# uber/aresdb

Hardware: AMD Instinct MI355X
Metric: rows/sec, 1B-row filter -> group-by-agg (whole job) (higher is better)
Workload: dtype u32 keys / f64 sums; 1 GPU; C3: filter d1<90 -> dims [floor(ts,3600), d1, d2, d3] (4 x uint32) -> SUM(m float32 -> float64) via HashReduce, validity bitmaps with 1% nulls, shard resident in HBM; rows_per_gpu=1000000000, batch_rows=67108864, batches=15, streams_per_query=2, parallelism=1 shard(s), one per GPU

## Files before the change

aresdb_amd/abi.py:

```python
import ctypes as C
import os

_HERE = os.path.dirname(os.path.abspath(__file__))
REPO_ROOT = os.path.dirname(_HERE)
LIB_DIR = os.environ.get("ARES_LIB_DIR") or os.path.join(_HERE, "lib")

AGGR_SUM_UNSIGNED, AGGR_SUM_SIGNED, AGGR_SUM_FLOAT = 1, 2, 3
AGGR_MIN_UNSIGNED, AGGR_MIN_SIGNED, AGGR_MIN_FLOAT = 4, 5, 6
AGGR_MAX_UNSIGNED, AGGR_MAX_SIGNED, AGGR_MAX_FLOAT = 7, 8, 9
AGGR_HLL, AGGR_AVG_FLOAT = 10, 11

(Bool, Int8, Uint8, Int16, Uint16, Int32, Uint32, Float32, Int64, Uint64, Float64, GeoPoint,
 UUID) = range(13)
ConstInt, ConstFloat, ConstGeoPoint, ConstUUID = range(4)
(Negate, Not, BitwiseNot, IsNull, IsNotNull, Noop, GetWeekStart, GetMonthStart, GetQuarterStart,
 GetYearStart, GetDayOfMonth, GetDayOfYear, GetMonthOfYear, GetQuarterOfYear, GetHLLValue,
 ArrayLength) = range(16)
(And, Or, Equal, NotEqual, LessThan, LessThanOrEqual, GreaterThan, GreaterThanOrEqual, Plus, Minus,
 Multiply, Divide, Mod, BitwiseAnd, BitwiseOr, BitwiseXor, Floor, ArrayContains,
 ArrayElementAt) = range(19)
(VectorPartyInput, ScratchSpaceInput, ConstantInput, ForeignColumnInput,
 ArrayVectorPartyInput) = range(5)
ScratchSpaceOutput, MeasureOutput, DimensionOutput = range(3)
NUM_DIM_WIDTH = 5
# ... 231 lines not shown
        return _check(getattr(self, "_" + sym)(*args))

    def mem_driver_calls(self, device=0):
        if not hasattr(self._mem, "AresMemDriverCalls"):
            return None
        m, f, t = C.c_size_t(0), C.c_size_t(0), C.c_size_t(0)
        self._mem.AresMemDriverCalls.argtypes = [C.c_int, C.POINTER(C.c_size_t), C.POINTER(C.c_size_t), C.POINTER(C.c_size_t)]
        self._mem.AresMemDriverCalls.restype = None
        self._mem.AresMemDriverCalls(device, C.byref(m), C.byref(f), C.byref(t))
        return {"mallocs": m.value, "frees": f.value, "trims": t.value}

    def rtc_wait(self):
        if not hasattr(self._algo, "AresRtcWait"):
            return None
        c = (C.c_long * 3)()
        self._algo.AresRtcWait.argtypes, self._algo.AresRtcWait.restype = [C.POINTER(C.c_long)], C.c_size_t
        n = self._algo.AresRtcWait(c)
        return {"kernels": int(n), "compiles": int(c[0]), "disk_hits": int(c[1]), "evictions": int(c[2])}

    def reload_env(self):
        if hasattr(self._algo, "AresReloadEnv"):
            self._algo.AresReloadEnv.argtypes, self._algo.AresReloadEnv.restype = [], None
            self._algo.AresReloadEnv()

    def flags(self):
        return self._mem.GetFlags()

    @property
    def has_fused_select(self):
        return hasattr(self._algo, "AresFusedFilterSelect")

    def fused_filter_select(self, query, batch_rows, limit, out_keys, stream=None, device=0):
        fn = self._algo.AresFusedFilterSelect
        fn.argtypes = [C.POINTER(FusedSelect), C.c_int, C.c_int, DimensionVector, _S, _I]
        fn.restype = CGoCallResHandle
        return _check(fn(C.byref(query), int(batch_rows), int(limit), out_keys, stream, device))

    def select_stats(self):
        c = (C.c_ulonglong * 4)()
        self._algo.AresSelectStats.argtypes, self._algo.AresSelectStats.restype = [C.POINTER(C.c_ulonglong)], None
        self._algo.AresSelectStats(c)
        return {"batches": int(c[0]), "declined": int(c[1]), "tiles": int(c[2]), "rows": int(c[3])}

    @property
    def has_fused_join_select(self):
        return hasattr(self._algo, "AresFusedFilterJoinSelect")

    def fused_filter_join_select(self, query, batch_rows, limit, out_keys, stream=None, device=0):
        fn = self._algo.AresFusedFilterJoinSelect
        fn.argtypes = [C.POINTER(FusedJoinSelect), C.c_int, C.c_int, DimensionVector, _S, _I]
        fn.restype = CGoCallResHandle
        return _check(fn(C.byref(query), int(batch_rows), int(limit), out_keys, stream, device))

    def select_join_stats(self):
        c = (C.c_ulonglong * 5)()
        self._algo.AresSelectJoinStats.argtypes, self._algo.AresSelectJoinStats.restype = [C.POINTER(C.c_ulonglong)], None
        self._algo.AresSelectJoinStats(c)
        return {"batches": int(c[0]), "declined": int(c[1]), "tiles": int(c[2]), "rows": int(c[3]), "probed": int(c[4])}

    @property
    def has_join_columns(self):
        return hasattr(self._algo, "AresJoinColumnsRun")

    def join_column_bytes(self, rows, dtype):
        fn = self._algo.AresJoinColumnBytes
        fn.argtypes, fn.restype = [C.c_int, C.c_int], C.c_size_t
        return int(fn(int(rows), int(dtype)))

    def join_columns_run(self, query, batch_rows, stream=None, device=0):
        fn = self._algo.AresJoinColumnsRun
        fn.argtypes = [C.POINTER(JoinColumns), C.c_int, C.POINTER(VectorPartySlice), _S, _I]
        fn.restype = CGoCallResHandle
        slices = (VectorPartySlice * 4)()
        res = _check(fn(C.byref(query), int(batch_rows), slices, stream, device))
        assert res == batch_rows
        return slices

    def join_column_stats(self):
        c = (C.c_ulonglong * 4)()
        self._algo.AresJoinColumnStats.argtypes, self._algo.AresJoinColumnStats.restype = [C.POINTER(C.c_ulonglong)], None
        self._algo.AresJoinColumnStats(c)
        return {"batches": int(c[0]), "declined": int(c[1]), "rows": int(c[2]), "probed": int(c[3])}

    def select_run_stats(self):
        c = (C.c_ulonglong * 2)()
        self._algo.AresSelectRunStats.argtypes, self._algo.AresSelectRunStats.restype = [C.POINTER(C.c_ulonglong)], None
        self._algo.AresSelectRunStats(c)
        return {"rejected": int(c[0]), "staged": int(c[1])}

    def profiler_enable(self, on=True):
        self._algo.AresProfilerEnable(1 if on else 0)

    def profiler_report(self):
        need = self._algo.AresProfilerReport(None, 0)
        buf = C.create_string_buffer(need + 16)
        self._algo.AresProfilerReport(buf, need + 16)
        out = {}
        for line in buf.value.decode().splitlines():
            name, launches, ms = line.rsplit(" ", 2)
            out[name] = (int(launches), float(ms))
        return out

    def device_alloc(self, nbytes, device=0):
        return self.call("DeviceAllocate", max(int(nbytes), 1), device)

    def device_free(self, ptr, device=0):
        self.call("DeviceFree", ptr, device)

    def h2d(self, dst, src_buf, nbytes, stream=None, device=0):
        self.call("AsyncCopyHostToDevice", dst, src_buf, nbytes, stream, device)

    def d2h(self, dst_buf, src, nbytes, stream=None, device=0):
        self.call("AsyncCopyDeviceToHost", dst_buf, src, nbytes, stream, device)

    def wait(self, stream=None, device=0):
        self.call("WaitForCudaStream", stream, device)


def hip_library_paths():
    return os.path.join(LIB_DIR, "libalgorithm.so"), os.path.join(LIB_DIR, "libmem.so")


def load_hip_backend():
    if not os.environ.get("ARES_NO_TORCH"):
        import torch
    algo, mem = hip_library_paths()
    return Backend("hip", algo, mem, device_memory=True)
```

aresdb_amd/csrc/algo/common.hpp:

```cpp
#pragma once

#include <hip/hip_runtime.h>

#include <atomic>
#include <chrono>
#include <cstdint>
#include <cstdio>
#include <cstdlib>
#include <cstring>
#include <stdexcept>
#include <string>

#include "ares_algorithm.h"

namespace ares {

class AlgorithmError : public std::runtime_error {
 public:
  explicit AlgorithmError(const std::string &m) : std::runtime_error(m) {}
};

void slow_trace(const char *what, double ms);
bool hr_trace_enabled();
class SlowScope {
 public:
  explicit SlowScope(const char *what) : what_(what), t0_(std::chrono::steady_clock::now()) {}
  ~SlowScope() {
    const double ms = std::chrono::duration<double, std::milli>(std::chrono::steady_clock::now() - t0_).count();
    if (ms > 5.0) slow_trace(what_, ms);
  }
  SlowScope(const SlowScope &) = delete;
  SlowScope &operator=(const SlowScope &) = delete;

 private:
  const char *what_;
  std::chrono::steady_clock::time_point t0_;
};
inline void hip_check(hipError_t e, const char *what) {
  if (e != hipSuccess) {
    (void)hipGetLastError();
    throw AlgorithmError(std::string("ERROR: ") + what + ": " + hipGetErrorString(e));
  }
}

template <class F>
inline void hip_check_timed(F &&call, const char *what) {
  SlowScope slow(what);
  hip_check(call(), what);
}
#define hip_check(expr, what) hip_check_timed([&]() -> hipError_t { return (expr); }, what)

extern void (*g_memNoteActivity)();
inline void mem_note_activity() {
  if (g_memNoteActivity) g_memNoteActivity();
}
inline void check_launch(const char *what) {
  mem_note_activity();
  hip_check(hipGetLastError(), what);
}

void flush_deferred(int device);
bool fuse_pending_into_hash_reduce(int device, hipStream_t stream, const DimensionVector &in, const uint8_t *inValues,
                                   const DimensionVector &out, uint8_t *outValues, int valueBytes, int length, int aggFunc,
                                   int *groups);
void invalidate_filter_journal(int device, const uint32_t *indexVector);
bool global_table_forced();
bool deferral_hooks_active();
void grouped_note_write(int device, const void *ptr, size_t bytes);
void grouped_note_write(int device, const DimensionVector &v);
void grouped_materialize_for_read(int device, const void *ptr, size_t bytes);
void grouped_trim(int device);
void flush_deferred_for_inputs(int device, const void *a, size_t aBytes, const void *b, size_t bBytes);
void flush_deferred_for_vector(int device, const DimensionVector &v, const void *values, size_t valueBytes);
void drop_skipped_outputs(int device, const void *a, size_t aBytes, const void *b, size_t bBytes);

bool defer_fill(int device, hipStream_t stream, void *dst, size_t bytes, uint64_t pattern, int unit);
bool pending_fill_exact(int device, const void *dst, size_t bytes, uint64_t *pattern, int *unit);
bool pending_fill_tail(int device, const void *base, int width, int length, int *prev, uint64_t *pattern);
void retire_fills_for_write(int device, const void *ptr, size_t bytes);
void materialize_fills_for_read(int device, const void *ptr, size_t bytes);
void launch_pending_writers(int device, const void *ptr, size_t bytes);
bool virtual_iota_peek(int device, const uint32_t *indexVector, int n, bool consume = false);
void materialize_index_vector(int device, const uint32_t *indexVector);
void settle_dimension_vector(int device, const DimensionVector &v, bool rowsOnly = false);
void temp_stats(size_t *handedOut, size_t *cached);

struct CallStream {
  hipStream_t stream;
  bool known;
};
extern thread_local CallStream t_callStream;
class CallStreamScope {
 public:
  CallStreamScope(void *stream, const char *entry) : saved_(t_callStream), slow_(entry) {
    t_callStream = CallStream{reinterpret_cast<hipStream_t>(stream), true};
  }
  ~CallStreamScope() { t_callStream = saved_; }
  CallStreamScope(const CallStreamScope &) = delete;
  CallStreamScope &operator=(const CallStreamScope &) = delete;

 private:
  CallStream saved_;
  SlowScope slow_;
};

#define ARES_ABI_BEGIN_NOFLUSH(device)                 \
  CGoCallResHandle resHandle = {nullptr, nullptr};     \
  try {                                                \
    ares::hip_check(hipSetDevice(device), "hipSetDevice");  \
    ares::CallStreamScope callStreamScope_(cudaStream, __func__);  \
    ares::mem_note_activity();                                      \
    (void)ares::deferral_hooks_active();

#define ARES_ABI_BEGIN(device)     \
  ARES_ABI_BEGIN_NOFLUSH(device)   \
  ares::flush_deferred(device);

#define ARES_ABI_END(name)                                            \
  }                                                                   \
  catch (std::exception & e) {                                        \
    fprintf(stderr, "Exception happened when doing %s: %s\n", name, e.what()); \
    resHandle.pStrErr = strdup(e.what());                             \
  }                                                                   \
  return resHandle;

extern std::atomic<uint32_t> g_envGeneration;
template <typename T>
class EnvSwitch {
 public:
  EnvSwitch(const char *name, T (*parse)(const char *)) : name_(name), parse_(parse) {}
  T get() {
    const uint32_t g = g_envGeneration.load(std::memory_order_acquire);
    if (gen_.load(std::memory_order_acquire) != g) {
      value_.store(parse_(getenv(name_)), std::memory_order_relaxed);
      gen_.store(g, std::memory_order_release);
    }
    return value_.load(std::memory_order_relaxed);
  }

 private:
  const char *name_;
  T (*parse_)(const char *);
  std::atomic<uint32_t> gen_{0};
  std::atomic<T> value_{};
};

inline void *int_result(int64_t v) { return reinterpret_cast<void *>(static_cast<intptr_t>(v)); }

// ... 66 lines not shown
```

aresdb_amd/csrc/algo/hash_reduce.hip:

```cpp
#include <hip/hip_runtime.h>

#include "aggregate.hpp"
#include "common.hpp"
#include "device_model.hpp"
#include "dim_layout.hpp"
#include "hash_reduce_lds.hpp"

namespace ares {

constexpr int kBlock = 256;
constexpr uint64_t kEmptyKey = ~0ull;

__global__ __launch_bounds__(kBlock) void hash_table_init_kernel(uint64_t *keys, uint8_t *values, uint64_t capacity,
                                                                 AggSpec a) {
  for (uint64_t s = static_cast<uint64_t>(blockIdx.x) * kBlock + threadIdx.x; s < capacity;
       s += static_cast<uint64_t>(gridDim.x) * kBlock) {
    keys[s] = kEmptyKey;
    if (a.width == 8) reinterpret_cast<uint64_t *>(values)[s] = a.identity;
    else reinterpret_cast<uint32_t *>(values)[s] = static_cast<uint32_t>(a.identity);
  }
}

__device__ __forceinline__ uint64_t find_or_claim(uint64_t *keys, uint64_t mask, uint32_t h, uint32_t row) {
  const uint64_t mine = (static_cast<uint64_t>(h) << 32) | row;
// ... 13 lines not shown
  }
}

__global__ __launch_bounds__(kBlock) void hash_insert_kernel(const uint8_t *dimValues, DimLayoutD L, size_t capacity,
                                                             const uint8_t *inputValues, AggSpec a, uint64_t *keys,
                                                             uint8_t *values, uint64_t mask, int length) {
  for (int64_t i64 = static_cast<int64_t>(blockIdx.x) * kBlock + threadIdx.x; i64 < length;
       i64 += static_cast<int64_t>(gridDim.x) * kBlock) {
    const uint32_t row = static_cast<uint32_t>(i64);
    Murmur32Stream ms(0);
    hash_dim_row(ms, dimValues, L, capacity, row);
    const uint32_t h = ms.finish();
    const uint64_t slot = find_or_claim(keys, mask, h, row);
    aggregate_slot(values + slot * a.width, inputValues + static_cast<size_t>(a.width) * row, a);
  }
}

constexpr int kExItems = 16;
__global__ __launch_bounds__(kBlock) void hash_extract_kernel(const uint64_t *keys, const uint8_t *values,
                                                              uint64_t tableSize, const uint8_t *dimIn, uint8_t *dimOut,
                                                              DimLayoutD L, size_t capacity, uint8_t *outputValues,
                                                              AggSpec a, uint32_t *counter) {
  __shared__ uint32_t sWave[kBlock / 64];
  __shared__ uint32_t sBase;
  const int lane = threadIdx.x & 63, wave = threadIdx.x >> 6;
  const uint64_t tileSlots = static_cast<uint64_t>(kBlock) * kExItems;
  for (uint64_t base = blockIdx.x * tileSlots; base < tableSize; base += gridDim.x * tileSlots) {
    uint64_t k[kExItems];
    uint32_t cnt = 0;
#pragma unroll
    for (int it = 0; it < kExItems; it++) {
      const uint64_t s = base + static_cast<uint64_t>(it) * kBlock + threadIdx.x;
      k[it] = s < tableSize ? keys[s] : kEmptyKey;
      cnt += k[it] != kEmptyKey;
    }
    uint32_t incl = cnt;
#pragma unroll
    for (int off = 1; off < 64; off <<= 1) {
      const uint32_t t = __shfl_up(incl, off);
      if (lane >= off) incl += t;
    }
    if (lane == 63) sWave[wave] = incl;
    __syncthreads();
    if (threadIdx.x == 0) {
      uint32_t total = 0;
      for (int w = 0; w < kBlock / 64; w++) {
        const uint32_t c = sWave[w];
        sWave[w] = total;
        total += c;
      }
      sBase = total ? atomicAdd(counter, total) : 0u;
    }
    __syncthreads();
    uint32_t dst = sBase + sWave[wave] + incl - cnt;
#pragma unroll
    for (int it = 0; it < kExItems; it++) {
      if (k[it] == kEmptyKey) continue;
      const uint64_t s = base + static_cast<uint64_t>(it) * kBlock + threadIdx.x;
      copy_dim_row(dimIn, capacity, dimOut, capacity, L, static_cast<uint32_t>(k[it]), dst);
      if (a.width == 8) reinterpret_cast<uint64_t *>(outputValues)[dst] = reinterpret_cast<const uint64_t *>(values)[s];
      else reinterpret_cast<uint32_t *>(outputValues)[dst] = reinterpret_cast<const uint32_t *>(values)[s];
      dst++;
    }
    __syncthreads();
  }
}

}

using namespace ares;

namespace ares {
bool global_table_forced() {
  static EnvSwitch<bool> forced("ARES_HASH_REDUCE", [](const char *e) { return e && strcmp(e, "global") == 0; });
  return forced.get();
}
}

extern "C" CGoCallResHandle HashReduce(DimensionVector inputKeys, uint8_t *inputValues, DimensionVector outputKeys,
                                       uint8_t *outputValues, int valueBytes, int length,
                                       enum AggregateFunction aggFunc, void *cudaStream, int device) {
  ARES_ABI_BEGIN_NOFLUSH(device)
  hipStream_t stream = reinterpret_cast<hipStream_t>(cudaStream);
  if (length > 0) {
    settle_dimension_vector(device, inputKeys);
    const DimLayoutD inLayout = make_dim_layout(inputKeys.NumDimsPerDimWidth);
    const size_t cap = inputKeys.VectorCapacity > 0 ? static_cast<size_t>(inputKeys.VectorCapacity) : 0;
    materialize_fills_for_read(device, inputKeys.DimValues, static_cast<size_t>(inLayout.rowBytes) * cap);
    materialize_fills_for_read(device, inputValues, static_cast<size_t>(valueBytes) * length);
    retire_fills_for_write(device, outputKeys.DimValues, static_cast<size_t>(inLayout.rowBytes) * cap);
    retire_fills_for_write(device, outputValues, static_cast<size_t>(valueBytes) * length);
  }
  {
    const DimLayoutD outLayout = make_dim_layout(outputKeys.NumDimsPerDimWidth);
    drop_skipped_outputs(device, outputKeys.DimValues,
                         static_cast<size_t>(outLayout.rowBytes) * (inputKeys.VectorCapacity > 0 ? inputKeys.VectorCapacity : 0),
                         outputValues, static_cast<size_t>(valueBytes) * (length > 0 ? length : 0));
  }
  int fusedGroups = 0;
  if (length > 0 && fuse_pending_into_hash_reduce(device, stream, inputKeys, inputValues, outputKeys, outputValues,
                                                  valueBytes, length, aggFunc, &fusedGroups)) {
    resHandle.res = int_result(fusedGroups);
    return resHandle;
  }
  {
    const DimLayoutD layout = make_dim_layout(inputKeys.NumDimsPerDimWidth);
    flush_deferred_for_inputs(device, inputKeys.DimValues, static_cast<size_t>(layout.rowBytes) * inputKeys.VectorCapacity,
                              inputValues, static_cast<size_t>(valueBytes) * (length > 0 ? length : 0));
  }
  const AggSpec a = make_agg_spec(aggFunc, valueBytes);
  int groups = -1;
  if (length > 0 && hash_reduce_lds_supported(a) && !global_table_forced())
    groups = hash_reduce_lds(device, inputKeys, inputValues, outputKeys, outputValues, a, length, stream);
  if (groups >= 0) {
    resHandle.res = int_result(groups);
  } else if (length > 0) {
    const DimLayoutD L = make_dim_layout(inputKeys.NumDimsPerDimWidth);
    grouped_note_write(device, outputValues, static_cast<size_t>(a.width) * length);
    grouped_note_write(device, outputKeys.DimValues, static_cast<size_t>(L.rowBytes) * inputKeys.VectorCapacity);
    uint64_t tableSize = 1024;
    while (tableSize < 2ull * static_cast<uint64_t>(length)) tableSize <<= 1;
    StreamBuffer keyBuf(tableSize * 8, stream), valBuf(tableSize * a.width, stream), counter(16, stream);
    hip_check(hipMemsetAsync(counter.get(), 0, 16, stream), "hipMemsetAsync");
    const int initGrid = capped_grid(static_cast<int64_t>((tableSize + kBlock - 1) / kBlock), 256 * 16);
    ARES_LAUNCH("hash_table_init_kernel", hash_table_init_kernel, initGrid, kBlock, stream, keyBuf.as<uint64_t>(),
                       valBuf.as<uint8_t>(), tableSize, a);
    const int grid = capped_grid((static_cast<int64_t>(length) + kBlock - 1) / kBlock, 256 * 16);
    ARES_LAUNCH("hash_insert_kernel", hash_insert_kernel, grid, kBlock, stream, inputKeys.DimValues, L,
                       static_cast<size_t>(inputKeys.VectorCapacity), inputValues, a, keyBuf.as<uint64_t>(),
                       valBuf.as<uint8_t>(), tableSize - 1, length);
    const int exGrid = capped_grid(static_cast<int64_t>((tableSize + kBlock * kExItems - 1) / (kBlock * kExItems)), 256 * 8);
    ARES_LAUNCH("hash_extract_kernel", hash_extract_kernel, exGrid, kBlock, stream, keyBuf.as<uint64_t>(),
                       valBuf.as<uint8_t>(), tableSize, inputKeys.DimValues, outputKeys.DimValues, L,
                       static_cast<size_t>(inputKeys.VectorCapacity), outputValues, a, counter.as<uint32_t>());
    uint32_t groups = 0;
    read_back_u32(counter.as<uint32_t>(), &groups, 1, stream);
    mem_note_dim_rows(device, outputKeys, 0, groups);
    mem_note_write(device, outputValues, static_cast<size_t>(a.width) * groups);
    resHandle.res = int_result(groups);
  }
  ARES_ABI_END("HashReduce")
}
```

aresdb_amd/csrc/algo/hash_reduce_lds.hip:

```cpp
#include <hip/hip_runtime.h>

#include <atomic>
#include <functional>
#include <map>
#include <mutex>
#include <string>
#include <unordered_map>

#include <memory>
#include <mutex>
#include <vector>

#include "aggregate.hpp"
#include "common.hpp"
#include "device_model.hpp"
#include "ares_extensions.h"
#include "dim_layout.hpp"
#include "fast_eval.hpp"
#include "hash_reduce_lds.hpp"
#include "hr_kernels.hpp"
#include "hr_rtc.hpp"
#include "sort_reduce_fused.hpp"

namespace ares {
// ... 599 lines not shown
    if (imageMode == 1) imageOut = take_image(device);
    if (prevSize > 0) grouped_materialize_for_read(device, prevValues, static_cast<size_t>(mw) * prevSize);
  }
  if (imageMode && !imageOut) {
    imageMode = 0;
    knownOut = 0;
    if (prevSize > 0) grouped_materialize_for_read(device, prevValues, static_cast<size_t>(mw) * prevSize);
  }
  {
    if (hr_trace_enabled())
      fprintf(stderr, "fused_hash_reduce_run: batch %d prev %d partBits %d | found %d (state: size %d partBits %d ranges %d image %d lazy %d) grouped %d "
                      "| lean %d table %d compact %d narrow %d -> image mode %d knownOut %u\n",
              batchRows, prevSize, partBits, found ? 1 : 0, found ? prev.size : -1, found ? prev.partBits : -1, found && prev.ranges ? 1 : 0,
              found && prev.image ? 1 : 0, found && prev.lazyValues ? 1 : 0, grouped ? 1 : 0, lean ? 1 : 0, table ? 1 : 0, compact ? 1 : 0,
              narrow ? 1 : 0, imageMode, knownOut);
  }
  if (narrow && !imageMode) {
    narrowMerge = rtc_lookup(device, rtc_spec_merge(plan, nd, partBits, a, widen, wantLean && compact,
                                                    wantTable || (prevSize > 0 && !grouped)));
    if (!narrowMerge) return kFusedUnavailable;
  }
  if (narrow && !(wantLean ? lean : table)) return kFusedUnavailable;
  bool launched = false;
  for (;;) {
    const bool prevToA = narrow && prevSize > 0 && !grouped && imageMode != 2;
    if (narrow && !imageMode) {
      narrowMerge = rtc_lookup(device, rtc_spec_merge(plan, nd, partBits, a, widen, lean && compact, table || prevToA));
      if (!narrowMerge) return launched ? -1 : kFusedUnavailable;
      if (table) tableMerge = narrowMerge;
    }
    launched = true;
    const int streams = batchRows > 0 ? (lean ? rtc_scan_grid(batchRows) : table ? 0 : grid_for(batchRows)) : 0;
    Regions r;
    {
      SlowScope slow("make_regions");
      const int64_t rowsA = !lean ? length : (prevSize > 0 && !grouped && imageMode != 2) ? prevSize : 0;
      make_regions(r, partBits, rowsA, batchRows, streams, lean ? 4 : 3, stream,
                   !lean ? 0 : compact ? static_cast<int>(kCompactLineRecords) : 8);
    }
    Workspace &ws = r.ws;
    ws.widen = widen;
    ws.chunkRows = static_cast<uint32_t>(chunkTiles) * 4096u;
    ws.rowBase = static_cast<uint32_t>(prevSize);
    ws.prevRanges = (grouped && imageMode != 2) ? prev.ranges.get() : nullptr;
    ws.outRanges = outRanges;
    Workspace wsPrev = ws;
    wsPrev.streams = 0;
    RtcKernel leanMerge = imageMode ? imageMerge
                          : narrow  ? (lean ? narrowMerge : nullptr)
                          : (lean && (prevSize == 0 || grouped)) ? rtc_lookup(device, rtc_spec_merge(plan, nd, partBits, a, widen, compact)) : nullptr;
    RtcImageArgs imageArgs{nullptr, nullptr, nullptr, nullptr, 0u};
    if (imageMode) {
      imageArgs.in = imageMode == 2 ? prev.image.get() : nullptr;
      imageArgs.inCount = imageMode == 2 ? image_counts(prev.image.get()) : nullptr;
      imageArgs.out = imageOut.get();
      imageArgs.outCount = image_counts(imageOut.get());
      imageArgs.knownOut = knownOut;
    }
    const RtcImageArgs *imagePtr = imageMode ? &imageArgs : nullptr;
    if (prevToA) {
      const DimLayoutD prevLayout = make_dim_layout(prevKeys.NumDimsPerDimWidth);
      const int64_t tiles = (static_cast<int64_t>(prevSize) + kTileRows - 1) / kTileRows;
      ARES_LAUNCH("hr_partition_kernel", hr_partition_kernel, static_cast<int>(tiles < 256 ? tiles : 256), kThreads, stream,
                  prevKeys.DimValues, prevLayout, prevCapacity, prevValues, a, prevSize, wsPrev);
    }
    if (outRanges && !leanMerge && !tableMerge) hip_check(hipMemsetAsync(outRanges, 0, kRangesBytes, stream), "hipMemsetAsync");
#define ARES_FUSED_CASE(ND)                                                                                            \
  case ND:                                                                                                             \
    if (prevSize > 0 && !grouped && !narrow && imageMode != 2) {                                                       \
      if (mw == 8)                                                                                                     \
        ARES_LAUNCH("hr_partition4_kernel", (hr_partition4_kernel<ND, 8>), grid_for(prevSize), kThreads, stream,        \
                    prevKeys.DimValues, prevCapacity, prevValues, 0u, a, prevSize, wsPrev, 0);                         \
      else                                                                                                             \
        ARES_LAUNCH("hr_partition4_kernel", (hr_partition4_kernel<ND, 4>), grid_for(prevSize), kThreads, stream,        \
                    prevKeys.DimValues, prevCapacity, prevValues, 0u, a, prevSize, wsPrev, 0);                         \
    }                                                                                                                  \
    if (batchRows > 0 && lean)                                                                                         \
      rtc_scan_launch(lean, leanKind, plan, static_cast<uint32_t>(prevSize), batchRows, ws, stream);                   \
    else if (batchRows > 0 && table)                                                                                   \
      rtc_scan_launch(table, RTC_SCAN_TABLE, plan, static_cast<uint32_t>(prevSize), batchRows, ws, stream);            \
    else if (batchRows > 0)                                                                                            \
      ARES_LAUNCH("hr_fused_scan_kernel", hr_fused_scan_kernel<ND>, streams, kThreads, stream, plan,                   \
                  static_cast<uint32_t>(prevSize), a, batchRows, ws);                                                  \
    if (leanMerge || tableMerge)                                                                                       \
      rtc_merge_launch(leanMerge ? leanMerge : tableMerge, plan, prevKeys.DimValues, prevCapacity, prevValues,         \
                       static_cast<uint32_t>(prevSize), outKeys.DimValues, outCapacity, outValues, ws, stream, imagePtr, \
                       result_slot());                                                                                 \
    else if (lean)                                                                                                     \
      ARES_LAUNCH("hr_fused_merge_kernel", (hr_fused_merge_kernel<ND, 4>), numParts, kThreads, stream, plan,            \
                  prevKeys.DimValues, prevCapacity, prevValues, static_cast<uint32_t>(prevSize), outKeys.DimValues,    \
                  outCapacity, outValues, a, ws);                                                                      \
    else                                                                                                               \
      ARES_LAUNCH("hr_fused_merge_kernel", (hr_fused_merge_kernel<ND, 3>), numParts, kThreads, stream, plan,            \
                  prevKeys.DimValues, prevCapacity, prevValues, static_cast<uint32_t>(prevSize), outKeys.DimValues,    \
                  outCapacity, outValues, a, ws);                                                                      \
    break;
    switch (nd) {
      ARES_FUSED_CASE(1) ARES_FUSED_CASE(2) ARES_FUSED_CASE(3) ARES_FUSED_CASE(4)
      default:
        if (batchRows > 0 && lean) rtc_scan_launch(lean, leanKind, plan, static_cast<uint32_t>(prevSize), batchRows, ws, stream);
        else if (batchRows > 0 && table) rtc_scan_launch(table, RTC_SCAN_TABLE, plan, static_cast<uint32_t>(prevSize), batchRows, ws, stream);
        rtc_merge_launch(leanMerge ? leanMerge : tableMerge, plan, prevKeys.DimValues, prevCapacity, prevValues, static_cast<uint32_t>(prevSize),
                         outKeys.DimValues, outCapacity, outValues, ws, stream, imagePtr, result_slot());
        break;
    }
    {
      SlowScope slow("read_result");
      res = ((leanMerge || tableMerge) && result_slot()) ? read_result_pinned(stream) : read_result(ws, stream);
    }
    if (imageMode == 2) res.groups += static_cast<uint32_t>(prevSize);
    if (imageMode == 2) {
      if (res.groups > knownOut) mem_note_dim_rows(device, outKeys, knownOut, res.groups - knownOut);
    } else {
      mem_note_dim_rows(device, outKeys, 0, res.groups);
      mem_note_write(device, outValues, static_cast<size_t>(mw) * res.groups);
    }
    if ((narrow || imageMode == 2) && res.needGeneric) {
      r.buf->mark_idle();
      return -1;
    }
    if (imageMode == 1 && res.needGeneric) imageMode = 0;
    if (leanMerge && res.needGeneric && !res.overflow && !(grouped && res.stale)) {
      hip_check(hipMemsetAsync(ws.outCount, 0, 4 * sizeof(uint32_t), stream), "hipMemsetAsync");
      if (outRanges) hip_check(hipMemsetAsync(outRanges, 0, kRangesBytes, stream), "hipMemsetAsync");
      switch (nd) {
#define ARES_FUSED_REMERGE(ND)                                                                                         \
  case ND:                                                                                                             \
    ARES_LAUNCH("hr_fused_merge_kernel", (hr_fused_merge_kernel<ND, 4>), numParts, kThreads, stream, plan,              \
                prevKeys.DimValues, prevCapacity, prevValues, static_cast<uint32_t>(prevSize), outKeys.DimValues,      \
                outCapacity, outValues, a, ws);                                                                        \
    break;
        ARES_FUSED_REMERGE(1) ARES_FUSED_REMERGE(2) ARES_FUSED_REMERGE(3) ARES_FUSED_REMERGE(4)
#undef ARES_FUSED_REMERGE
      }
      res = read_result(ws, stream);
      mem_note_dim_rows(device, outKeys, 0, res.groups);
      mem_note_write(device, outValues, static_cast<size_t>(mw) * res.groups);
    }
#undef ARES_FUSED_CASE
    r.buf->mark_idle();
    if (grouped && res.stale) {
      grouped_note_write(device, prevKeys.DimValues, slots.row_bytes() * prevCapacity);
      grouped = false;
      imageMode = 0;
      continue;
    }
    if (res.overflow && lean && grow_record_stream_slack()) continue;
    break;
  }
  if (res.overflow) {
    return -1;
  }
  fused_note_first_batch(shape, static_cast<int>(res.groups));
  if (shape && !lean && !table) {
    if (static_cast<int>(res.groups) >= lean_min_groups()) {
      (void)rtc_lookup(device, rtc_spec_scan(plan, nd, partBits, compact));
      (void)rtc_lookup(device, rtc_spec_merge(plan, nd, partBits, a, widen, compact));
    } else {
      (void)rtc_lookup(device, rtc_spec_table_scan(plan, nd, partBits, a, widen));
    }
  }
  if (outRanges) {
    GroupedState s{device, outKeys.DimValues, outValues, outCapacity, slots, mw, static_cast<int>(res.groups), partBits, outRangesRef};
    if (imageMode == 2) {
      s.ranges = nullptr;
      s.image = imageOut;
      s.lineage = prev.lineage;
      s.gen = ++g_generation;
      s.parentGen = prev.gen;
      s.lazyValues = true;
    } else if (imageMode == 1) {
      s.image = imageOut;
      s.lineage = ++g_lineage;
      s.gen = ++g_generation;
    }
    if (res.groups > 0) grouped_register(s);
  }
  return static_cast<int>(res.groups);
}

namespace {

struct NotFusable : std::runtime_error {
  explicit NotFusable(const std::string &why) : std::runtime_error("not fusable: " + why) {}
// ... 78 lines not shown
```

aresdb_amd/csrc/algo/hll.hip:

```cpp
#include <dlfcn.h>
#include <hip/hip_runtime.h>

#include <atomic>
#include <cstring>
#include <string>

#include "ares_extensions.h"
#include "common.hpp"
#include "dim_layout.hpp"
#include "hash_reduce_lds.hpp"
#include "hr_kernels.hpp"
#include "hr_rtc.hpp"
#include "lookback.hpp"
#include "sort_reduce.hpp"

namespace ares {

namespace {

constexpr int kBlock = 256;

__device__ __forceinline__ bool hll_less(uint64_t h1, uint32_t v1, uint64_t h2, uint32_t v2) {
  return h1 == h2 ? v1 > v2 : h1 < h2;
}
// ... 541 lines not shown
  DimScanParams dp;
  dp.regStart = hp.regStart;
  dp.dims = dims;
  dp.registers = totals[1];
  dp.numTiles = dimTiles;
  dp.regCount = regCount;
  dp.ticket = reinterpret_cast<unsigned int *>(base2);
  dp.error = reinterpret_cast<uint32_t *>(base2) + 1;
  dp.status = reinterpret_cast<uint64_t *>(base2 + 64);
  dp.offsets = dp.status + dimTiles;
  ARES_LAUNCH("hll_dim_scan_kernel", hll_dim_scan_kernel, capped_grid(dimTiles), kBlock, stream, dp);
  uint32_t tail[2] = {0, 0};
  read_back_u32(reinterpret_cast<const uint32_t *>(dp.offsets + dims), tail, 2, stream);
  uint32_t err = 0;
  read_back_u32(dp.error, &err, 1, stream);
  if (err) throw AlgorithmError("ERROR: HyperLogLog: inter-tile scan timed out");
  const size_t total = static_cast<size_t>(tail[0]) | (static_cast<size_t>(tail[1]) << 32);

  uint8_t *hllVector = static_cast<uint8_t *>(result_alloc(total));
  *hllVectorPtr = hllVector;
  *hllVectorSizePtr = total;
  hip_check(hipMemsetAsync(hllVector, 0, total, stream), "hipMemsetAsync");
  ARES_LAUNCH("hll_write_kernel", hll_write_kernel, capped_grid((static_cast<int64_t>(n) + kBlock - 1) / kBlock, 256 * 8),
              kBlock, stream, cur.HashValues, curValues, n, hp.entryDim, hp.entryReg, hp.regStart, regCount, dp.offsets,
              hllVector);
  hip_check(hipMemcpyAsync(cur.IndexVector, hp.headIndex, sizeof(uint32_t) * static_cast<size_t>(dims),
                           hipMemcpyDeviceToDevice, stream), "hipMemcpyAsync");
  return dims;
}

int hyperloglog(const DimensionVector &prev, const DimensionVector &cur, uint32_t *prevValues, uint32_t *curValues,
                int prevResultSize, int curBatchSize, bool isLastBatch, uint8_t **hllVectorPtr,
                size_t *hllVectorSizePtr, uint16_t **regCountPtr, hipStream_t stream) {
  if (prevResultSize < 0 || curBatchSize < 0) throw std::invalid_argument("HyperLogLog: negative size");
  if (static_cast<int64_t>(prevResultSize) + curBatchSize >= (1ll << 30))
    throw std::invalid_argument("HyperLogLog supports up to 2^30 - 1 entries per call");
  const DimLayoutD L = make_dim_layout(cur.NumDimsPerDimWidth);
  const size_t capacity = static_cast<size_t>(cur.VectorCapacity);
  const int P = prevResultSize, n = curBatchSize;

  int runs = 0;
  if (n > 0) runs = hll_preagg_batch(prev, cur, prevValues, curValues, P, n, stream);
  if (n > 0 && runs < 0) {
    StreamBuffer positions(sizeof(uint32_t) * static_cast<size_t>(n), stream);
    sort_rows(prev.DimValues, L, capacity, cur.IndexVector, curValues, cur.HashValues, positions.as<uint32_t>(), true,
              n, stream);
    runs = hll_reduce_sorted(cur.HashValues, positions.as<uint32_t>(), cur.IndexVector, curValues, prev.HashValues + P,
                             prev.IndexVector + P, prevValues + P, n, stream);
  }
  int resSize = P + runs;
  if (resSize > 0) {
    const int tiles = (resSize + kMergeTile - 1) / kMergeTile;
    StreamBuffer split(sizeof(int) * (static_cast<size_t>(tiles) + 1), stream);
    ARES_LAUNCH("hll_merge_split_kernel", hll_merge_split_kernel, (tiles + 1 + kBlock - 1) / kBlock, kBlock, stream,
                prev.HashValues, prevValues, P, runs, tiles, split.as<int>());
    ARES_LAUNCH("hll_merge_kernel", hll_merge_kernel, tiles, kBlock, stream, prev.HashValues, prevValues,
                prev.IndexVector, P, runs, split.as<int>(), cur.HashValues, curValues, cur.IndexVector);
    if (isLastBatch)
      resSize = make_hll_vector(cur, curValues, resSize, hllVectorPtr, hllVectorSizePtr, regCountPtr, stream);
    ARES_LAUNCH("hll_gather_dims_kernel", hll_gather_dims_kernel,
                capped_grid((static_cast<int64_t>(resSize) + kBlock - 1) / kBlock, 256 * 8), kBlock, stream, prev.DimValues,
                cur.DimValues, make_dim_layout(prev.NumDimsPerDimWidth), static_cast<size_t>(prev.VectorCapacity),
                cur.IndexVector, resSize);
  }
  return resSize;
}

}

}

using namespace ares;

extern "C" void AresHllPreaggStats(unsigned long long *counters) {
  if (!counters) return;
  for (int i = 0; i < 4; i++) counters[i] = g_preaggStats[i].load(std::memory_order_relaxed);
}

extern "C" CGoCallResHandle HyperLogLog(DimensionVector prevDimOut, DimensionVector curDimOut, uint32_t *prevValuesOut,
                                        uint32_t *curValuesOut, int prevResultSize, int curBatchSize, bool isLastBatch,
                                        uint8_t **hllVectorPtr, size_t *hllVectorSizePtr,
                                        uint16_t **hllDimRegIDCountPtr, void *cudaStream, int device) {
  ARES_ABI_BEGIN(device)
  settle_dimension_vector(device, prevDimOut);
  settle_dimension_vector(device, curDimOut);
  {
    const size_t capV = static_cast<size_t>(prevDimOut.VectorCapacity > curDimOut.VectorCapacity ? prevDimOut.VectorCapacity : curDimOut.VectorCapacity);
    materialize_fills_for_read(device, prevValuesOut, 4 * capV);
    materialize_fills_for_read(device, curValuesOut, 4 * capV);
  }
  flush_deferred_for_vector(device, prevDimOut, nullptr, 0);
  flush_deferred_for_vector(device, curDimOut, nullptr, 0);
  grouped_note_write(device, prevDimOut);
  grouped_note_write(device, curDimOut);
  {
    mem_note_vector_all(device, prevDimOut);
    mem_note_vector_all(device, curDimOut);
    const size_t cap = static_cast<size_t>(prevDimOut.VectorCapacity > curDimOut.VectorCapacity ? prevDimOut.VectorCapacity
                                                                                                    : curDimOut.VectorCapacity);
    mem_note_write(device, prevValuesOut, 4 * cap);
    mem_note_write(device, curValuesOut, 4 * cap);
  }
  resHandle.res = reinterpret_cast<void *>(static_cast<intptr_t>(
      hyperloglog(prevDimOut, curDimOut, prevValuesOut, curValuesOut, prevResultSize, curBatchSize, isLastBatch,
                  hllVectorPtr, hllVectorSizePtr, hllDimRegIDCountPtr, reinterpret_cast<hipStream_t>(cudaStream))));
  ARES_ABI_END("HyperLogLog")
}
```

aresdb_amd/csrc/algo/sort_reduce.hip:

```cpp
#include <hip/hip_runtime.h>

#include "aggregate.hpp"
#include "common.hpp"
#include "device_model.hpp"
#include "dim_layout.hpp"
#include "lookback.hpp"
#include "sort_reduce_fused.hpp"

namespace ares {

constexpr int kBlock = 256;
constexpr int kWaves = kBlock / 64;

__global__ __launch_bounds__(kBlock) void sort_hash_hist_kernel(const uint8_t *dimValues, DimLayoutD L, size_t capacity,
                                                                const uint32_t *indexVector, uint64_t *hashes, int n,
                                                                uint32_t *globalHist ,
                                                                const uint32_t *hllValues, uint32_t *iotaOut) {
  __shared__ uint32_t sHist[8 * 256];
  for (int i = threadIdx.x; i < 8 * 256; i += kBlock) sHist[i] = 0;
  __syncthreads();
  for (int64_t i = static_cast<int64_t>(blockIdx.x) * kBlock + threadIdx.x; i < n;
       i += static_cast<int64_t>(gridDim.x) * kBlock) {
    Murmur128Stream ms(0);
    hash_dim_row(ms, dimValues, L, capacity, indexVector[i]);
// ... 826 lines not shown
    if (constRows) {
      uint64_t folded = constBits;
      if (a.op == OP_SUM) folded = (a.width == 8 ? constBits * static_cast<uint64_t>(constRows)
                                                 : static_cast<uint64_t>(static_cast<uint32_t>(constBits) * constRows));
      acc = combine_bits(a, acc, folded);
      any = true;
    }
  }
#pragma unroll
  for (int off = 32; off > 0; off >>= 1) {
    const uint64_t other = __shfl_xor(static_cast<unsigned long long>(acc), off);
    acc = combine_bits(a, acc, other);
  }
  if (__ballot(any) && (threadIdx.x & 63) == 0) aggregate_slot(out, reinterpret_cast<const uint8_t *>(&acc), a);
}

static bool reduce_without_dimensions(int device, const DimensionVector &in, const uint8_t *inputValues, const DimensionVector &out,
                                      uint8_t *outputValues, int valueBytes, int length, int aggFunc, hipStream_t stream, int *groups) {
  if (length <= 0) return false;
  const DimLayoutD L = make_dim_layout(in.NumDimsPerDimWidth), LO = make_dim_layout(out.NumDimsPerDimWidth);
  if (L.numDims != 0 || LO.numDims != 0 || aggFunc == AGGR_AVG_FLOAT) return false;
  AggSpec a;
  try {
    a = make_agg_spec(aggFunc, valueBytes);
  } catch (std::exception &) {
    return false;
  }
  if (!(a.vtype == V_U32 || a.vtype == V_I32 || a.vtype == V_U64 || a.vtype == V_I64)) return false;
  uint64_t hashPattern = 0;
  int hashUnit = 0;
  if (!in.HashValues || !in.IndexVector || !virtual_iota_peek(device, in.IndexVector, length) ||
      !pending_fill_exact(device, in.HashValues, 8ull * static_cast<size_t>(length), &hashPattern, &hashUnit) || hashUnit != 8)
    return false;
  int prev = length;
  uint64_t c = 0;
  if (!pending_fill_tail(device, inputValues, a.width, length, &prev, &c)) prev = length;
  if (prev > 0) {
    launch_pending_writers(device, inputValues, static_cast<size_t>(a.width) * prev);
    materialize_fills_for_read(device, inputValues, static_cast<size_t>(a.width) * prev);
  }
  retire_fills_for_write(device, outputValues, static_cast<size_t>(a.width));
  if (out.IndexVector) retire_fills_for_write(device, out.IndexVector, 4);
  mem_note_write(device, outputValues, static_cast<size_t>(a.width));
  if (out.IndexVector) mem_note_write(device, out.IndexVector, 4);
  (void)virtual_iota_peek(device, in.IndexVector, length, true);
  ARES_LAUNCH("fill_identity_kernel", fill_identity_kernel, 1, kBlock, stream, outputValues, a, 1);
  const int grid = capped_grid((static_cast<int64_t>(prev) + kBlock * 8 - 1) / (kBlock * 8), 256 * 4);
  ARES_LAUNCH("reduce_all_kernel", reduce_all_kernel, grid, kBlock, stream, inputValues, prev, a, c, static_cast<uint32_t>(length - prev),
              outputValues, out.IndexVector);
  *groups = 1;
  return true;
}

}

using namespace ares;

extern "C" {

CGoCallResHandle Sort(DimensionVector keys, int length, void *cudaStream, int device) {
  ARES_ABI_BEGIN_NOFLUSH(device)
  if (length > 0 && make_dim_layout(keys.NumDimsPerDimWidth).numDims == 0 && keys.HashValues && keys.IndexVector &&
      virtual_iota_peek(device, keys.IndexVector, length) &&
      defer_fill(device, reinterpret_cast<hipStream_t>(cudaStream), keys.HashValues, 8ull * static_cast<size_t>(length), empty_row_hash(), 8))
    return resHandle;
  if (define_lazy_sort(device, reinterpret_cast<hipStream_t>(cudaStream), keys, length)) return resHandle;
  const bool lazyVectors = lazy_vector_sort_candidate(device, keys, length);
  flush_deferred(device);
  settle_dimension_vector(device, keys, lazyVectors);
  flush_deferred_for_vector(device, keys, nullptr, 0);
  if (lazyVectors && define_lazy_sort_vectors(device, reinterpret_cast<hipStream_t>(cudaStream), keys, length)) return resHandle;
  if (length > 0) {
    mem_note_write(device, keys.HashValues, 8ull * static_cast<size_t>(length));
    mem_note_write(device, keys.IndexVector, 4ull * static_cast<size_t>(length));
  }
  sort_impl(keys, length, reinterpret_cast<hipStream_t>(cudaStream));
  ARES_ABI_END("Sort")
}

CGoCallResHandle Reduce(DimensionVector inputKeys, uint8_t *inputValues, DimensionVector outputKeys,
                        uint8_t *outputValues, int valueBytes, int length, enum AggregateFunction aggFunc,
                        void *cudaStream, int device) {
  ARES_ABI_BEGIN_NOFLUSH(device)
  {
    int groups = 0;
    if (reduce_without_dimensions(device, inputKeys, inputValues, outputKeys, outputValues, valueBytes, length, aggFunc,
                                  reinterpret_cast<hipStream_t>(cudaStream), &groups)) {
      resHandle.res = int_result(groups);
      return resHandle;
    }
  }
  {
    int groups = 0;
    if (length > 0 && fuse_pending_into_sort_reduce(device, reinterpret_cast<hipStream_t>(cudaStream), inputKeys, inputValues, outputKeys,
                                                    outputValues, valueBytes, length, aggFunc, &groups)) {
      resHandle.res = int_result(groups);
      return resHandle;
    }
  }
  flush_deferred(device);
  settle_dimension_vector(device, inputKeys);
  settle_dimension_vector(device, outputKeys);
  retire_fills_for_write(device, outputValues, static_cast<size_t>(valueBytes) * (length > 0 ? length : 0));
  flush_deferred_for_vector(device, inputKeys, inputValues, static_cast<size_t>(valueBytes) * (length > 0 ? length : 0));
  grouped_note_write(device, outputKeys);
  grouped_note_write(device, outputValues, static_cast<size_t>(valueBytes) * (length > 0 ? length : 0));
  drop_skipped_outputs(device, outputKeys.DimValues, 1, outputValues, static_cast<size_t>(valueBytes) * (length > 0 ? length : 0));
  if (length > 0) {
    mem_note_dim_rows(device, outputKeys, 0, static_cast<size_t>(length));
    mem_note_write(device, outputKeys.IndexVector, 4ull * static_cast<size_t>(length));
    mem_note_write(device, outputValues, static_cast<size_t>(valueBytes) * static_cast<size_t>(length));
  }
  resHandle.res = int_result(reduce_impl(inputKeys, inputValues, outputKeys, outputValues, valueBytes, length, aggFunc,
                                         reinterpret_cast<hipStream_t>(cudaStream)));
  ARES_ABI_END("Reduce")
}

CGoCallResHandle Expand(DimensionVector inputKeys, DimensionVector outputKeys, uint32_t *baseCounts,
                        uint32_t *indexVector, int indexVectorLen, int outputOccupiedLen, void *cudaStream, int device) {
  ARES_ABI_BEGIN(device)
  settle_dimension_vector(device, inputKeys);
  settle_dimension_vector(device, outputKeys);
  materialize_index_vector(device, indexVector);
  flush_deferred_for_vector(device, inputKeys, nullptr, 0);
  grouped_note_write(device, outputKeys);
  mem_note_vector_all(device, outputKeys);
  resHandle.res = int_result(expand_impl(inputKeys, outputKeys, baseCounts, indexVector, indexVectorLen,
                                         outputOccupiedLen, reinterpret_cast<hipStream_t>(cudaStream)));
  ARES_ABI_END("Expand")
}

}
```

aresdb_amd/csrc/algo/transform.hip:

```cpp
#include <hip/hip_runtime.h>

#include <dlfcn.h>

#include <algorithm>
#include <map>
#include <memory>
#include <mutex>
#include <string>
#include <vector>

#include "ares_extensions.h"

#include "binding.hpp"
#include "common.hpp"
#include "device_model.hpp"
#include "dim_layout.hpp"
#include "fast_eval.hpp"
#include "hash_reduce_lds.hpp"
#include "lookback.hpp"
#include "sort_reduce_fused.hpp"

#include "transform_kernels.hpp"

namespace ares {


static void materialize_sort(const uint32_t *indexVector);
static void drop_sort(const uint32_t *indexVector);
namespace {
struct ByteRange {
  const uint8_t *lo, *hi;
  bool overlaps(const ByteRange &o) const { return lo < o.hi && o.lo < hi; }
};
ByteRange range_of(const void *ptr, size_t bytes) {
  const uint8_t *lo = static_cast<const uint8_t *>(ptr);
  return ByteRange{lo, lo + (bytes ? bytes : 1)};
}
template <typename Visit>
void column_ranges(const FastOperands &f, uint32_t colRows, Visit &&visit) {
  visit(range_of(f.vals, fast_value_bytes(f, colRows)));
  if (f.nulls) visit(range_of(f.nulls, (static_cast<uint64_t>(colRows) + f.bitOff + 7) / 8 + 2));
}
bool column_overlaps(const FastOperands &f, uint32_t colRows, const ByteRange &r) {
  bool hit = false;
  column_ranges(f, colRows, [&](const ByteRange &c) { hit = hit || c.overlaps(r); });
  return hit;
}
struct PendingQueue {
  MultiJobs jobs;
  uint32_t colRows[kMaxMultiJobs];
  const uint32_t *idx = nullptr;
  int n = 0;
  std::vector<ByteRange> reads, writes;
  bool overWait = false;
  std::vector<std::shared_ptr<StreamBuffer>> keep;
  const uint32_t *sortIdx = nullptr;
};
struct DeferState;
DeferState &state_of(int device);
thread_local DeferState *t_state = nullptr;
thread_local std::vector<hipStream_t> t_syncAfterUnlock;
struct DeferLock {
  std::unique_lock<std::mutex> lock;
  explicit DeferLock(int device);
  void unlock() {
    if (lock.owns_lock()) {
      t_state = nullptr;
      lock.unlock();
    }
    drain();
  }
  static void drain() {
    std::vector<hipStream_t> todo;
    todo.swap(t_syncAfterUnlock);
    for (size_t i = 0; i < todo.size(); i++) {
      bool seen = false;
      for (size_t j = 0; j < i; j++) seen = seen || todo[j] == todo[i];
      if (!seen) hip_check(hipStreamSynchronize(todo[i]), "hipStreamSynchronize");
    }
  }
  ~DeferLock() noexcept(false) {
    if (lock.owns_lock()) {
      t_state = nullptr;
      lock.unlock();
    }
    if (std::uncaught_exceptions() == 0) drain();
    else t_syncAfterUnlock.clear();
// ... 100 lines not shown
struct PendingFill {
  hipStream_t stream;
  size_t bytes;
  uint64_t pattern;
  int unit;
  bool streamGone = false;
  const uint32_t *sortIdx = nullptr;
};

struct PendingSort {
  hipStream_t stream;
  DimensionVector keys;
  int length;
  bool reduced = false;
  bool fromVectors = false;
  DimensionVector outKeys;
  uint8_t *inValues = nullptr, *outValues = nullptr;
  int valueBytes = 0, aggFunc = 0, groups = 0;
  bool constMeasure = false;
  uint8_t *fillAt = nullptr;
  PendingFill fill;
};

void hook_on_wait(int device, void *stream);
uintptr_t hook_on_free(int device, void *ptr, size_t bytes);
void hook_on_access(int device, const void *ptr, size_t bytes);
void hook_on_write(int device, const void *ptr, size_t bytes);
void hook_on_stream_destroy(int device, void *stream);
void hook_trim(int device);

bool defer_available() {
  static const bool ok = [] {
    const char *e = getenv("ARES_DEFER");
    if (e && e[0] == '0') return false;
    Dl_info info;
    if (!dladdr(reinterpret_cast<void *>(&AresFlushDeferred), &info) || !info.dli_fname) return false;
    std::string path(info.dli_fname);
    const size_t slash = path.rfind('/');
    path = (slash == std::string::npos ? std::string(".") : path.substr(0, slash)) + "/libmem.so";
    void *h = dlopen(path.c_str(), RTLD_NOW | RTLD_NOLOAD);
    if (!h) return false;
    auto set = reinterpret_cast<void (*)(void (*)(int))>(dlsym(h, "AresMemSetFlushHook"));
    if (!set) return false;
    set(&AresFlushDeferred);
    const char *fuse = getenv("ARES_FUSE");
    auto setHooks = reinterpret_cast<void (*)(const AresDeferralHooks *)>(dlsym(h, "AresMemSetDeferralHooks"));
    auto release = reinterpret_cast<void (*)(int, uintptr_t)>(dlsym(h, "AresMemReleaseHeld"));
    g_fuseEnabled = !(fuse && fuse[0] == '0');
    if (setHooks && release) {
      static const AresDeferralHooks hooks = {&AresFlushDeferred, &hook_on_wait, &hook_on_free, &hook_on_access};
      g_releaseHeld = release;
      setHooks(&hooks);
    }
    auto setAux = reinterpret_cast<void (*)(const AresMemAuxHooks *)>(dlsym(h, "AresMemSetAuxHooks"));
    if (setAux) {
      static const AresMemAuxHooks aux = {sizeof(AresMemAuxHooks), &hook_on_write, &hook_on_stream_destroy, &hook_trim};
      setAux(&aux);
    }
    g_memTrimCache = reinterpret_cast<void (*)(int)>(dlsym(h, "AresMemTrimCache"));
    g_memNoteWrite = reinterpret_cast<void (*)(int, const void *, size_t)>(dlsym(h, "AresMemNoteWrite"));
    auto track = reinterpret_cast<void (*)()>(dlsym(h, "AresMemEnableWriteTracking"));
    if (g_memNoteWrite && track) track();
    else g_memNoteWrite = nullptr;
    g_memNoteActivity = reinterpret_cast<void (*)()>(dlsym(h, "AresMemNoteActivity"));
    auto share = reinterpret_cast<void (*)()>(dlsym(h, "AresMemEnableActivityTracking"));
    if (g_memNoteActivity && share) share();
    else g_memNoteActivity = nullptr;
    return true;
  }();
  return ok;
}
bool fuse_available() { return defer_available() && g_releaseHeld != nullptr && g_fuseEnabled; }
}
bool deferral_hooks_active() { return defer_available() && g_releaseHeld != nullptr; }
namespace {

struct ErrorCheck {
  hipStream_t stream;
  hipEvent_t done;
  uint32_t *pinned;
  std::shared_ptr<StreamBuffer> ws;
};

struct DeferState {
  std::mutex mutex;
  int device = -1;
  std::map<hipStream_t, PendingQueue> pending;
  std::map<hipStream_t, PendingQueue> limbo;
  std::map<const uint32_t *, FilterJournal> journals;
  std::map<const uint32_t *, PendingCompact> compactions;
  std::map<hipStream_t, FilterHistory> filterHistory;
  uint64_t filterGeneration = 0;
  std::map<uint32_t *, PendingIota> iotas;
  std::map<uint8_t *, PendingFill> fills;
  std::map<const uint32_t *, PendingSort> sorts;
  std::map<hipStream_t, std::vector<RunExpansion>> expansions;
  std::vector<ErrorCheck> errorChecks;
  std::vector<uint32_t *> errorSlots;
  bool errorSeen = false;
};
constexpr int kMaxDevices = 64;
DeferState &state_of(int device) {
  static struct States {
    DeferState of[kMaxDevices];
    States() {
      for (int d = 0; d < kMaxDevices; d++) of[d].device = d;
    }
  } states;
  if (device < 0 || device >= kMaxDevices) throw std::invalid_argument("device index out of range");
  return states.of[device];
}
DeferLock::DeferLock(int device) : lock(state_of(device).mutex, std::defer_lock) {
  {
    SlowScope slow("wait for the device's deferral lock");
    lock.lock();
  }
  t_state = &state_of(device);
}

void watch_error_word(hipStream_t stream, const uint32_t *errorDev, std::shared_ptr<StreamBuffer> ws) {
  ErrorCheck c;
  c.stream = stream;
  c.ws = std::move(ws);
  if (!t_state->errorSlots.empty()) {
    c.pinned = t_state->errorSlots.back();
    t_state->errorSlots.pop_back();
  } else {
    hip_check(hipHostMalloc(reinterpret_cast<void **>(&c.pinned), sizeof(uint32_t), hipHostMallocPortable), "hipHostMalloc");
  }
  hip_check(hipEventCreateWithFlags(&c.done, hipEventDisableTiming), "hipEventCreate");
  *c.pinned = 0;
  hip_check(hipMemcpyAsync(c.pinned, errorDev, sizeof(uint32_t), hipMemcpyDeviceToHost, stream), "hipMemcpyAsync");
  hip_check(hipEventRecord(c.done, stream), "hipEventRecord");
  t_state->errorChecks.push_back(std::move(c));
}

bool retire_error_check(size_t i) {
  ErrorCheck &c = t_state->errorChecks[i];
  const bool failed = *c.pinned != 0;
  (void)hipEventDestroy(c.done);
  t_state->errorSlots.push_back(c.pinned);
  t_state->errorChecks[i] = std::move(t_state->errorChecks.back());
  t_state->errorChecks.pop_back();
  return failed;
}

void poll_error_words() {
  bool failed = t_state->errorSeen;
  t_state->errorSeen = false;
  for (size_t i = 0; i < t_state->errorChecks.size();) {
    if (hipEventQuery(t_state->errorChecks[i].done) == hipSuccess) {
      failed = retire_error_check(i) || failed;
    } else {
      (void)hipGetLastError();
      i++;
    }
  }
  if (failed) throw AlgorithmError("ERROR: filter: compaction wait timed out (reported by a deferred compaction)");
}

int pred_tiles(int n, int pad) {
  const int64_t numQuads = (static_cast<int64_t>(n) + pad + 3) / 4;
  return static_cast<int>((numQuads + kBlock * kPQ - 1) / (kBlock * kPQ));
}
CompactSpace clear_compact_space(const StreamBuffer &ws, int tiles, int passes, size_t extraWords, hipStream_t stream) {
  CompactSpace cs;
  cs.words = ws.as<uint32_t>();
  cs.tiles = tiles;
  cs.passes = passes;
  hip_check(hipMemsetAsync(cs.words, 0, CompactSpace::bytes(tiles, passes, extraWords), stream), "hipMemsetAsync");
  return cs;
}
void launch_compaction(const CompactSpace &cs, const uint8_t *pred, uint32_t *idx, bool virtualIdx, RecordID **recordIDVectors, int pad, int n,
                       hipStream_t stream) {
  ARES_LAUNCH("filter_scan_kernel", filter_scan_kernel, 1, 1024, stream, cs.tileCounts(), cs.tileOffsets(), cs.tiles, cs.total());
  const int cgrid = capped_grid((cs.tiles + kTilesPerTicket - 1) / kTilesPerTicket, 256 * 8);
  for (int pass = 0; pass < cs.passes; pass++) {
    CompactWorkspace cw;
    cw.ticket = cs.tickets() + pass;
// ... 749 lines not shown
  EvalParams p;
  SinkD s;
  CallTemps temps;
  build_params(ins, arity, stream, indexVector, baseCounts, startCount, functor, p, temps);
  const std::shared_ptr<StreamBuffer> decoded = decode_run_length_operand(device, stream, p.a, indexVector, baseCounts, startCount);
  bind_sink(output, baseCounts, s);
  if (s.type == SINK_MEASURE && s.baseCounts && indexVector) p.needRow = 1;
  if (s.type == SINK_DIM || s.type == SINK_MEASURE) {
    grouped_note_write(device, s.values, static_cast<size_t>(s.width) * n);
    if (s.nulls) grouped_note_write(device, s.nulls, static_cast<size_t>(n));
  }
  if (s.type == SINK_MEASURE && !s.baseCounts && arity == 1 && functor == Noop && p.a.type == OP_CONST && !is_wide(p.a.kind) &&
      s.agg != AGGR_AVG_FLOAT && (s.width == 4 || s.width == 8)) {
    uint64_t pattern = 0;
    if (constant_measure_bits(p, s, &pattern) && defer_fill(device, stream, s.values, static_cast<size_t>(s.width) * n, pattern, s.width))
      return n;
  }
  retire_fills_for_write(device, s.values, static_cast<size_t>(s.width) * n);
  if (s.nulls) retire_fills_for_write(device, s.nulls, static_cast<size_t>(n));
  FastOperands f;
  bool fast = fast_sink(s) && fast_operands(p, f, false);
  if (fast && s.type == SINK_DIM && s.width < 4 && !(f.rk == K_I32 || f.rk == K_U32)) fast = false;
  if (fast && s.type == SINK_MEASURE && s.agg == AGGR_AVG_FLOAT && !avg_hot_shape(f)) fast = false;
  if (fast && f.idx && virtual_iota(device, indexVector, n, false)) f.idx = nullptr;
  if (fast && (s.type == SINK_DIM || s.type == SINK_MEASURE) && defer_transform(device, stream, f, s, n, p.a.length, decoded)) return n;
  flush_deferred(device);
  materialize_index_vector(device, indexVector);
  note_sink(device, s, n);
  if (fast) {
    launch_fast_transform(f, s, n, stream);
  } else if (is_wide(p.a.kind)) {
    const int grid = capped_grid((static_cast<int64_t>(n) + kBlock - 1) / kBlock);
    ARES_LAUNCH("transform_wide_kernel", transform_wide_kernel, grid, kBlock, stream, p, s, n);
  } else if (foreign_gather_enabled() && p.arity == 1 && functor == Noop && p.a.type == OP_FOREIGN && !p.a.tz && !p.needRow && !s.baseCounts) {
    constexpr int ITEMS = 8;
    const int grid = capped_grid((static_cast<int64_t>(n) + kBlock * ITEMS - 1) / (kBlock * ITEMS), 256 * 16);
    ARES_LAUNCH("transform_foreign_kernel", transform_foreign_kernel<ITEMS>, grid, kBlock, stream, p, s, n);
  } else {
    constexpr int ITEMS = 4;
    const int grid = capped_grid((static_cast<int64_t>(n) + kBlock * ITEMS - 1) / (kBlock * ITEMS), 256 * 16);
    ARES_LAUNCH("transform32_kernel", transform32_kernel<ITEMS>, grid, kBlock, stream, p, s, n);
  }
  return n;
}

namespace {
int compute_units(int device) {
  static std::mutex mu;
  static std::map<int, int> known;
  std::lock_guard<std::mutex> lock(mu);
  auto it = known.find(device);
  if (it != known.end()) return it->second;
  int cus = 0;
  if (hipDeviceGetAttribute(&cus, hipDeviceAttributeMultiprocessorCount, device) != hipSuccess || cus < 1) {
    (void)hipGetLastError();
    cus = 256;
  }
  return known[device] = cus;
}
int resident_blocks(int device, const void *kernel, int blockSize) {
  static std::mutex mu;
  static std::map<std::pair<int, const void *>, int> known;
  std::lock_guard<std::mutex> lock(mu);
  auto it = known.find({device, kernel});
  if (it != known.end()) return it->second;
  int perCU = 0;
  if (hipOccupancyMaxActiveBlocksPerMultiprocessor(&perCU, kernel, blockSize, 0) != hipSuccess || perCU < 1) {
    (void)hipGetLastError();
    perCU = 4;
  }
  return known[{device, kernel}] = perCU * compute_units(device);
}

bool row_space_enabled() {
  static EnvSwitch<bool> on("ARES_FILTER_ROWSPACE", [](const char *e) { return !(e && e[0] == '0'); });
  return on.get();
}
bool same_column(const FastOperands &a, const FastOperands &b) { return a.vals == b.vals && a.nulls == b.nulls && a.bitOff == b.bitOff; }
bool same_filter(const FastOperands &a, const FastOperands &b) {
  return same_column(a, b) && a.akind == b.akind && a.arity == b.arity && a.functor == b.functor && a.I == b.I && a.bkind == b.bkind &&
         a.bbits == b.bbits && a.bok == b.bok;
}

bool row_space_eligible(int device, hipStream_t stream, const uint32_t *indexVector, int n, uint32_t colRows) {
  if (!fuse_available() || !row_space_enabled()) return false;
  DeferLock lock(device);
  auto j = t_state->journals.find(indexVector);
  if (j == t_state->journals.end() || !j->second.valid || j->second.stream != stream || j->second.start != 0 ||
      j->second.filters.size() >= static_cast<size_t>(kFusedFilters) || colRows < static_cast<uint32_t>(j->second.n0))
    return false;
  auto c = t_state->compactions.find(indexVector);
  if (j->second.filters.empty()) return n == j->second.n0 && c == t_state->compactions.end();
  return c != t_state->compactions.end() && !c->second.todo.empty() && c->second.stream == stream &&
         c->second.applied + c->second.todo.size() == j->second.filters.size() && c->second.lastCount == n;
}

int run_filter_rows(int device, hipStream_t stream, FastOperands f, uint32_t *indexVector, uint8_t *pred, int n, uint32_t colRows,
                    bool virtualIdx, const std::shared_ptr<StreamBuffer> &keep = nullptr) {
  f.idx = nullptr;
  f.pad = 0;
  f.streaming = 1;
  constexpr int kGridCap = 2048;
  static_assert(2 * kGridCap <= kPinnedWords, "the partial counts are read back in one copy");
  std::shared_ptr<StreamBuffer> bits1, bits2;
  int grid = 0;
  bool two = false;
  FastOperands g = f;
  uint64_t generation = 0;
  {
    DeferLock lock(device);
    auto ins = t_state->compactions.find(indexVector);
    {
      auto jr = t_state->journals.find(indexVector);
      const size_t journalled = (jr != t_state->journals.end() && jr->second.valid) ? jr->second.filters.size() : 0;
      const bool first = ins == t_state->compactions.end() && journalled == 1 && jr->second.n0 == n;
      const bool next = ins != t_state->compactions.end() && !ins->second.todo.empty() && ins->second.stream == stream &&
                        ins->second.applied + ins->second.todo.size() + 1 == journalled && ins->second.lastCount == n;
      if (!first && !next) return -1;
    }
    if (ins == t_state->compactions.end()) {
      PendingCompact fresh{};
      fresh.stream = stream;
      fresh.idx = indexVector;
      fresh.virtualIdx = virtualIdx;
      fresh.n0 = n;
      fresh.applied = 0;
      fresh.lastCount = n;
      ins = t_state->compactions.emplace(indexVector, fresh).first;
    }
    PendingCompact &c = ins->second;
    FilterHistory &h = t_state->filterHistory[stream];
    FilterShape shape{f.akind, f.functor, f.I, f.bkind, f.bbits, f.bok, !c.todo.empty() && same_column(c.todo.back().f, f)};
    const size_t k = h.current.size();
    h.current.push_back(shape);
    if (c.predicted.valid && same_filter(c.predicted.g, f)) {
      const int count = c.predicted.count;
      c.todo.push_back(LazyFilter{f, colRows, pred, n, keep});
      c.bits = c.predicted.bits;
      c.lastCount = count;
      c.predicted = PredictedFilter{};
      auto j = t_state->journals.find(indexVector);
      if (j != t_state->journals.end() && j->second.valid) j->second.lastCount = count;
      return count;
    }
    c.predicted = PredictedFilter{};
    if (k + 1 < h.previous.size() && h.previous[k].same_as(shape) && h.previous[k + 1].sameColumnAsPrevious &&
        h.previous[k + 1].akind == f.akind && c.applied + c.todo.size() + 2 <= static_cast<size_t>(kFusedFilters)) {
      const FilterShape &nx = h.previous[k + 1];
      g.functor = nx.functor;
      g.I = nx.I;
      g.bkind = nx.bkind;
      g.bbits = nx.bbits;
      g.bok = nx.bok;
      two = true;
    }
    const int tiles = pred_tiles(c.n0, 0);
    const bool hasIn = static_cast<bool>(c.bits);
    auto kernel = two ? (hasIn ? &filter_rows_kernel<true, true> : &filter_rows_kernel<true, false>)
                      : (hasIn ? &filter_rows_kernel<false, true> : &filter_rows_kernel<false, false>);
    {
      const int resident = resident_blocks(device, reinterpret_cast<const void *>(kernel), kBlock), cus = compute_units(device);
      const int perUnit = std::max(1, std::min(resident / cus - 1, 6));
      grid = capped_grid(tiles, std::min(kGridCap, cus * perUnit));
    }
    const size_t bitBytes = static_cast<size_t>(tiles) * kBlock * sizeof(uint16_t);
    bits1 = std::make_shared<StreamBuffer>(bitBytes, stream);
    if (two) bits2 = std::make_shared<StreamBuffer>(bitBytes, stream);
    uint32_t *hostPartials = reinterpret_cast<uint32_t *>(pinned_words());
    ARES_LAUNCH("filter_rows_kernel", kernel, grid, kBlock, stream, f, g,
                hasIn ? c.bits->as<uint16_t>() : static_cast<const uint16_t *>(nullptr), bits1->as<uint16_t>(),
                two ? bits2->as<uint16_t>() : static_cast<uint16_t *>(nullptr), c.n0, tiles, hostPartials);
    c.todo.push_back(LazyFilter{f, colRows, pred, n, keep});
    c.bits = bits1;
    c.lastCount = -1;
    generation = ++t_state->filterGeneration;
    c.generation = generation;
  }
  hip_check(hipStreamSynchronize(stream), "hipStreamSynchronize");
  const volatile uint32_t *parts = reinterpret_cast<const volatile uint32_t *>(pinned_words());
  uint32_t count = 0, count2 = 0;
  for (int b = 0; b < grid; b++) {
    count += parts[2 * b];
    count2 += parts[2 * b + 1];
  }
  {
    DeferLock lock(device);
    auto it = t_state->compactions.find(indexVector);
    if (it != t_state->compactions.end() && it->second.generation == generation) {
      it->second.lastCount = static_cast<int>(count);
      if (two) {
        it->second.predicted.valid = true;
        it->second.predicted.g = g;
        it->second.predicted.count = static_cast<int>(count2);
        it->second.predicted.bits = bits2;
      }
    }
    auto j = t_state->journals.find(indexVector);
    if (j != t_state->journals.end() && j->second.valid) j->second.lastCount = static_cast<int>(count);
  }
  return static_cast<int>(count);
}

bool prepare_filter(int device, hipStream_t stream, const EvalParams &p, uint32_t *indexVector, uint8_t *pred, int n,
                    int numForeignTables, const uint32_t *baseCounts, bool *virtualIdx) {
  bool rowSpace = false;
  *virtualIdx = false;
  FastOperands probe;
  if (!is_wide(p.a.kind) && indexVector != nullptr && numForeignTables == 0 && fast_operands(p, probe, true)) {
    *virtualIdx = virtual_iota(device, indexVector, n, true);
    rowSpace = baseCounts == nullptr && row_space_eligible(device, stream, indexVector, n, p.a.length);
  }
  if (rowSpace) flush_deferred_impl(device, nullptr, nullptr, indexVector);
  else flush_deferred(device);
  rowSpace = rowSpace && row_space_eligible(device, stream, indexVector, n, p.a.length);
  if (!rowSpace) mem_note_write(device, pred, static_cast<size_t>(n));
  materialize_index_vector(device, indexVector);
  return rowSpace;
}

int run_filter_two_phase(int device, hipStream_t stream, FastOperands f, uint32_t *indexVector, uint8_t *pred, int n,
                         RecordID **recordIDVectors, int numForeignTables, bool virtualIdx) {
  f.pad = static_cast<int>(reinterpret_cast<uintptr_t>(pred) & 3);
  const int tiles = pred_tiles(n, f.pad);
  const int passes = 1 + numForeignTables;
  constexpr int kPredGridCap = 256 * 16;
  static_assert(kPredGridCap <= kPinnedWords, "the partial counts are read back in one copy");
  const int predGrid = capped_grid(tiles, kPredGridCap);
  auto wsBuf = std::make_shared<StreamBuffer>(CompactSpace::bytes(tiles, passes, predGrid), stream);
  const CompactSpace cs = clear_compact_space(*wsBuf, tiles, passes, predGrid, stream);
  if (virtualIdx) f.idx = nullptr;
  const bool lazy = numForeignTables == 0 && journal_is_valid(device, indexVector);
  uint32_t *partials = cs.extra();
  ARES_LAUNCH("filter_pred_kernel", filter_pred_kernel, predGrid, kBlock, stream, f, pred, cs.tileCounts(), n, tiles,
              lazy ? partials : nullptr);
  if (lazy) {
    uint32_t parts[kPredGridCap];
    read_back_u32(partials, parts, predGrid, stream);
    uint32_t count = 0;
    for (int b = 0; b < predGrid; b++) count += parts[b];
    PendingCompact c;
    c.stream = stream;
    c.idx = indexVector;
    c.pred = pred;
    c.n = n;
    c.pad = f.pad;
    c.virtualIdx = virtualIdx;
    c.ws = wsBuf;
    c.space = cs;
    DeferLock lock(device);
    t_state->compactions[indexVector] = c;
    return static_cast<int>(count);
  }
  mem_note_write(device, indexVector, 4ull * static_cast<size_t>(n));
  for (int t = 0; t < numForeignTables; t++) mem_note_write(device, recordIDVectors[t], 8ull * static_cast<size_t>(n));
  launch_compaction(cs, pred, indexVector, virtualIdx, recordIDVectors, f.pad, n, stream);
  return read_compaction_total(cs, stream);
}

int run_filter_generic(int device, hipStream_t stream, EvalParams p, const ArrayD *arr, uint32_t *indexVector, uint8_t *pred, int n,
                       RecordID **recordIDVectors, int numForeignTables) {
  if (is_wide(p.a.kind)) {
    SinkD s;
    bind_pred_sink(pred, s);
    p.needRow = indexVector != nullptr;
    const int grid = capped_grid((static_cast<int64_t>(n) + kBlock - 1) / kBlock);
    if (arr)
      launch_array(*arr, s, n, stream);
    else
      ARES_LAUNCH("transform_wide_kernel", transform_wide_kernel, grid, kBlock, stream, p, s, n);
  }
  mem_note_write(device, indexVector, 4ull * static_cast<size_t>(n));
  for (int t = 0; t < numForeignTables; t++) mem_note_write(device, recordIDVectors[t], 8ull * static_cast<size_t>(n));
  const int numTiles = static_cast<int>((static_cast<int64_t>(n) + kFilterTile - 1) / kFilterTile);
  const int passes = 1 + numForeignTables;
  const size_t passBytes = 16 + sizeof(uint64_t) * static_cast<size_t>(numTiles);
  StreamBuffer wsBuf(passBytes * passes, stream);
  hip_check(hipMemsetAsync(wsBuf.get(), 0, passBytes * passes, stream), "hipMemsetAsync");
  const int grid = capped_grid(numTiles);
  uint32_t *totalDev = nullptr;
  for (int pass = 0; pass < passes; pass++) {
    uint8_t *base = wsBuf.as<uint8_t>() + passBytes * pass;
    ScanWorkspace ws;
    ws.ticket = reinterpret_cast<unsigned int *>(base);
    ws.total = reinterpret_cast<uint32_t *>(base + 4);
    ws.error = reinterpret_cast<uint32_t *>(wsBuf.as<uint8_t>() + 8);
    ws.status = reinterpret_cast<uint64_t *>(base + 16);
    if (pass == 0) {
      totalDev = ws.total;
      if (is_wide(p.a.kind)) {
        ARES_LAUNCH("filter_kernel<2>", filter_kernel<2>, grid, kBlock, stream, p, pred, indexVector,
                           static_cast<uint64_t *>(nullptr), ws, n, numTiles);
      } else {
        ARES_LAUNCH("filter_kernel<0>", filter_kernel<0>, grid, kBlock, stream, p, pred, indexVector,
                    static_cast<uint64_t *>(nullptr), ws, n, numTiles);
      }
    } else {
      ARES_LAUNCH("filter_kernel<1>", filter_kernel<1>, grid, kBlock, stream, p, pred, indexVector,
                  reinterpret_cast<uint64_t *>(recordIDVectors[pass - 1]), ws, n, numTiles);
    }
  }
  uint32_t result[2] = {0, 0};
  read_back_u32(totalDev, result, 2, stream);
  if (result[1]) throw AlgorithmError("ERROR: filter: inter-tile scan timed out");
  return static_cast<int>(result[0]);
}
}

static int run_filter(const InputVector *ins, int arity, uint32_t *indexVector, uint8_t *pred, int n,
                      RecordID **recordIDVectors, int numForeignTables, uint32_t *baseCounts, uint32_t startCount,
                      int functor, hipStream_t stream, int device) {
  if (numForeignTables < 0 || numForeignTables > 8) throw std::invalid_argument("only support up to 8 foreign tables");
  if (n <= 0) {
    flush_deferred(device);
    return 0;
  }
  EvalParams p;
  CallTemps temps;
  const bool isArray = ins[0].Type == ArrayVectorPartyInput;
  ArrayD arr;
  std::shared_ptr<StreamBuffer> decoded;
  if (isArray) {
    bind_array(ins, arity, functor, Bool, arr);
    memset(&p, 0, sizeof(p));
    p.a.kind = K_UUID;
  } else {
    build_params(ins, arity, stream, indexVector, baseCounts, startCount, functor, p, temps);
    decoded = decode_run_length_operand(device, stream, p.a, indexVector, baseCounts, startCount);
  }
  p.needRow = 1;
  bool virtualIdx = false;
  const bool rowSpace = prepare_filter(device, stream, p, indexVector, pred, n, numForeignTables, baseCounts, &virtualIdx);
  FastOperands f;
  const bool fast = !is_wide(p.a.kind) && indexVector != nullptr && fast_operands(p, f, true);
  if (fast && numForeignTables == 0 && baseCounts == nullptr)
    journal_filter(device, indexVector, &f, p.a.length, n, decoded);
  else
    journal_filter(device, indexVector, nullptr, 0, 0);
  if (rowSpace && fast && journal_is_valid(device, indexVector)) {
    const int counted = run_filter_rows(device, stream, f, indexVector, pred, n, p.a.length, virtualIdx, decoded);
    if (counted >= 0) return counted;
  }
  if (rowSpace) {
    mem_note_write(device, pred, static_cast<size_t>(n));
    DeferLock lock(device);
    run_compaction(indexVector);
  }
  if (fast) return run_filter_two_phase(device, stream, f, indexVector, pred, n, recordIDVectors, numForeignTables, virtualIdx);
  return run_filter_generic(device, stream, p, isArray ? &arr : nullptr, indexVector, pred, n, recordIDVectors, numForeignTables);
}

namespace {
bool touches(const std::vector<ByteRange> &v, const ByteRange &r) {
  for (const ByteRange &x : v)
    if (x.overlaps(r)) return true;
  return false;
}
bool journal_touched(const uint32_t *indexVector, const FilterJournal &j, const ByteRange &r, bool *indexOnly) {
  const bool idx = range_of(indexVector, 4ull * (j.n0 > 0 ? j.n0 : 1)).overlaps(r);
  bool cols = false;
  for (size_t k = 0; k < j.filters.size(); k++) cols = cols || column_overlaps(j.filters[k], j.colRows[k], r);
  if (indexOnly) *indexOnly = idx && !cols;
  return idx || cols;
}

struct DeviceGuard {
  int previous = -1;
  explicit DeviceGuard(int device) {
    if (hipGetDevice(&previous) != hipSuccess) previous = -1;
    if (previous != device) (void)hipSetDevice(device);
  }
  ~DeviceGuard() {
    if (previous >= 0) (void)hipSetDevice(previous);
  }
};

void hook_on_wait(int device, void *streamPtr) {
  hipStream_t stream = reinterpret_cast<hipStream_t>(streamPtr);
  try {
    DeviceGuard guard(device);
    DeferLock lock(device);
    for (auto it = t_state->iotas.begin(); it != t_state->iotas.end();) {
      it = (it->second.stream == stream && !it->second.consumed) ? write_iota(it) : std::next(it);
    }
    for (auto &kv : t_state->pending) {
      if (kv.first != stream || kv.second.jobs.count == 0 || kv.second.overWait) continue;
      PendingQueue &q = kv.second;
      bool keep = g_fuseEnabled;
      if (keep && q.idx) {
        auto j = t_state->journals.find(q.idx);
        keep = j != t_state->journals.end() && j->second.valid && j->second.stream == stream && j->second.start == 0;
        if (keep)
          for (size_t k = 0; k < j->second.filters.size(); k++)
            column_ranges(j->second.filters[k], j->second.colRows[k], [&](const ByteRange &c) { q.reads.push_back(c); });
      }
      if (keep)
        q.overWait = true;
      else
        launch_queue(kv.first, q);
    }
  } catch (std::exception &e) {
    fprintf(stderr, "Exception happened when handling a stream wait: %s\n", e.what());
  }
}

uintptr_t hook_on_free(int device, void *ptr, size_t bytes) {
  const ByteRange r = range_of(ptr, bytes);
  grouped_note_write(device, ptr, bytes);
  uintptr_t hold = 0;
  ReleaseSet released;
  try {
    DeviceGuard guard(device);
    DeferLock lock(device);
    for (auto it = t_state->sorts.begin(); it != t_state->sorts.end();) {
      if (sort_touches(it->second, r)) {
        drop_sort(it->first);
        it = t_state->sorts.begin();
      } else {
        ++it;
      }
    }
    for (auto it = t_state->iotas.begin(); it != t_state->iotas.end();) {
      const ByteRange v = range_of(it->first, 4ull * it->second.n);
      it = v.overlaps(r) ? t_state->iotas.erase(it) : std::next(it);
    }
    retire_fills(r, true);
    forget_run_expansions(r);
    for (auto it = t_state->journals.begin(); it != t_state->journals.end();) {
      const bool dead = journal_touched(it->first, it->second, r, nullptr);
      bool kept = false;
      if (dead)
        for (auto &kv : t_state->pending) kept = kept || (kv.second.jobs.count && kv.second.overWait && kv.second.idx == it->first);
      it = (dead && !kept) ? t_state->journals.erase(it) : std::next(it);
    }
    for (auto &kv : t_state->pending) {
      if (kv.second.jobs.count == 0) continue;
      if (touches(kv.second.writes, r)) {
        released.add(kv.first);
        launch_queue(kv.first, kv.second);
      } else if (touches(kv.second.reads, r)) {
        if (kv.second.overWait) {
          hold = hold_tag(kv.first);
        } else {
          released.add(kv.first);
          launch_queue(kv.first, kv.second);
        }
      }
    }
    for (auto it = t_state->compactions.begin(); it != t_state->compactions.end();) {
      if (!compaction_touches(it->second, r)) {
        ++it;
        continue;
      }
      const uint32_t *key = it->first;
      const hipStream_t owner = it->second.stream;
      bool waited = false, queued = false, skipped = false;
      for (auto &kv : t_state->pending)
        if (kv.second.jobs.count && kv.second.idx == key) (kv.second.overWait ? waited : queued) = true;
      for (auto &kv : t_state->limbo) skipped = skipped || kv.second.idx == key;
      if (waited || skipped) {
        hold = hold_tag(owner);
        ++it;
      } else if (queued) {
        for (auto &kv : t_state->pending)
          if (kv.second.jobs.count && kv.second.idx == key) {
            released.add(kv.first);
            launch_queue(kv.first, kv.second);
          }
        it = t_state->compactions.begin();
      } else if (range_of(it->second.idx, 4ull * (it->second.todo.empty() ? it->second.n : it->second.n0)).overlaps(r)) {
        it = t_state->compactions.erase(it);
      } else {
        run_compaction(key);
        it = t_state->compactions.begin();
      }
    }
    for (auto it = t_state->limbo.begin(); it != t_state->limbo.end();) {
      if (touches(it->second.writes, r)) {
        it = drop_limbo(it, &released);
      } else {
        if (touches(it->second.reads, r)) hold = hold_tag(it->first);
        ++it;
      }
    }
  } catch (std::exception &e) {
    fprintf(stderr, "Exception happened when handling a device free: %s\n", e.what());
  }
  released.run(device);
  return hold;
}

void hook_on_access(int device, const void *ptr, size_t bytes) {
  const ByteRange r = range_of(ptr, bytes);
  ReleaseSet released;
  try {
    DeviceGuard guard(device);
    grouped_materialize_for_read(device, ptr, bytes);
    DeferLock lock(device);
    for (auto it = t_state->iotas.begin(); it != t_state->iotas.end();) {
      const ByteRange v = range_of(it->first, 4ull * it->second.n);
      if (v.overlaps(r)) {
        t_syncAfterUnlock.push_back(it->second.stream);
        it = write_iota(it);
      } else {
        ++it;
      }
    }
    for (auto &kv : t_state->pending) {
      if (kv.second.jobs.count == 0) continue;
      if (touches(kv.second.writes, r) || touches(kv.second.reads, r)) {
        released.add(kv.first);
        launch_queue(kv.first, kv.second);
      }
    }
    forget_run_expansions(r);
    materialize_fills(&r, &t_syncAfterUnlock);
    materialize_limbo(&r, &released);
    for (auto it = t_state->compactions.begin(); it != t_state->compactions.end();) {
      if (compaction_touches(it->second, r)) {
        const hipStream_t cs = it->second.stream;
        run_compaction(it->first);
        t_syncAfterUnlock.push_back(cs);
        it = t_state->compactions.begin();
      } else {
        ++it;
      }
    }
    for (auto it = t_state->journals.begin(); it != t_state->journals.end();)
      it = journal_touched(it->first, it->second, r, nullptr) ? t_state->journals.erase(it) : std::next(it);
  } catch (std::exception &e) {
    fprintf(stderr, "Exception happened when handling a device copy: %s\n", e.what());
  }
  released.run(device);
}
}

namespace {
void hook_on_write(int device, const void *ptr, size_t bytes) { grouped_note_write(device, ptr, bytes); }

void hook_trim(int device) {
  try {
    DeviceGuard guard(device);
    stream_cache_trim(device);
    grouped_trim(device);
  } catch (std::exception &) {
  }
}

void hook_on_stream_destroy(int device, void *streamPtr) {
  hipStream_t stream = reinterpret_cast<hipStream_t>(streamPtr);
  try {
    DeviceGuard guard(device);
    {
      DeferLock lock(device);
      for (auto it = t_state->sorts.begin(); it != t_state->sorts.end();) {
        if (it->second.stream == stream) {
          drop_sort(it->first);
          it = t_state->sorts.begin();
        } else {
          ++it;
        }
      }
      t_state->pending.erase(stream);
      t_state->expansions.erase(stream);
      auto lim = t_state->limbo.find(stream);
      if (lim != t_state->limbo.end()) drop_limbo(lim, nullptr);
      for (auto it = t_state->journals.begin(); it != t_state->journals.end();)
        it = it->second.stream == stream ? t_state->journals.erase(it) : std::next(it);
      for (auto it = t_state->compactions.begin(); it != t_state->compactions.end();)
        it = it->second.stream == stream ? t_state->compactions.erase(it) : std::next(it);
      for (auto it = t_state->iotas.begin(); it != t_state->iotas.end();)
        it = it->second.stream == stream ? t_state->iotas.erase(it) : std::next(it);
      t_state->filterHistory.erase(stream);
      for (auto &kv : t_state->fills)
        if (kv.second.stream == stream) kv.second.streamGone = true;
      for (size_t i = 0; i < t_state->errorChecks.size();) {
        if (t_state->errorChecks[i].stream == stream) t_state->errorSeen = retire_error_check(i) || t_state->errorSeen;
        else i++;
      }
    }
    profiler_stream_gone(stream);
    if (g_releaseHeld) g_releaseHeld(device, hold_tag(stream));
    stream_cache_purge(device, stream);
  } catch (std::exception &e) {
    fprintf(stderr, "Exception happened when handling a stream destruction: %s\n", e.what());
  }
}
}

void launch_pending_writers(int device, const void *ptr, size_t bytes) {
  if (!ptr || bytes == 0 || !defer_available()) return;
  grouped_materialize_for_read(device, ptr, bytes);
  const ByteRange r = range_of(ptr, bytes);
  ReleaseSet released;
  {
    DeferLock lock(device);
    for (auto &kv : t_state->pending) {
      if (kv.second.jobs.count == 0 || !touches(kv.second.writes, r)) continue;
      if (kv.second.overWait) released.add(kv.first);
      launch_queue(kv.first, kv.second);
    }
    materialize_limbo(&r, &released);
  }
  released.run(device);
}

namespace {
bool match_jobs(const PendingQueue &pq, const DimensionVector &in, const DimLayoutD &L, int prev, int (&dimJob)[kFusedDims], int *measureJob) {
  const int nd = L.numDims;
  const size_t cap = static_cast<size_t>(in.VectorCapacity);
  if (nd < 1 || nd > kFusedDims || in.NumDimsPerDimWidth[0] || in.NumDimsPerDimWidth[1]) return false;
  if (pq.jobs.count != nd && pq.jobs.count != nd + 1) return false;
  for (int c = 0; c < kFusedDims; c++) dimJob[c] = -1;
  *measureJob = -1;
  for (int k = 0; k < pq.jobs.count; k++) {
    const SinkD &s = pq.jobs.s[k];
    if (s.type == SINK_MEASURE) {
      if (*measureJob >= 0 || s.baseCounts) return false;
      *measureJob = k;
      continue;
    }
    int d = -1;
    for (int c = 0; c < nd; c++)
      if (s.values == in.DimValues + static_cast<size_t>(L.valueOff[c]) * cap + static_cast<size_t>(L.width[c]) * prev &&
          s.nulls == in.DimValues + static_cast<size_t>(L.valueBytes) * cap + cap * c + prev && s.width == L.width[c])
        d = c;
    if (s.type != SINK_DIM || d < 0 || dimJob[d] >= 0) return false;
    dimJob[d] = k;
  }
  for (int c = 0; c < nd; c++)
    if (dimJob[c] < 0) return false;
  return true;
}
bool measure_job_matches(const SinkD &s, const uint8_t *measureRows, int valueBytes, int aggFunc) {
  return s.values == measureRows && s.width == valueBytes && s.agg == aggFunc &&
         !(valueBytes == 8 && s.identity != 0);
}
bool queue_survivors(const PendingQueue &pq, const FilterJournal **journal, int *n0) {
  *journal = nullptr;
  *n0 = pq.n;
  if (!pq.idx) return true;
  auto j = t_state->journals.find(pq.idx);
  if (j == t_state->journals.end() || !j->second.valid || j->second.start != 0) return false;
  *journal = &j->second;
  *n0 = j->second.n0;
  return true;
}
bool columns_cover(const uint32_t *colRows, size_t count, int n0) {
  for (size_t k = 0; k < count; k++)
    if (colRows[k] < static_cast<uint32_t>(n0)) return false;
  return true;
}
bool plan_from_queue(FusedPlanD &plan, const PendingQueue &pq, const DimLayoutD &L, const int (&dimJob)[kFusedDims], int measureJob, int valueBytes,
                     uint64_t constBits, int constDtype, const FilterJournal *journal, int n0) {
  const int nd = L.numDims;
  for (int c = 0; c < nd; c++) fused_plan_dim(plan, c, pq.jobs.f[dimJob[c]], pq.jobs.s[dimJob[c]], L.width[c]);
  if (measureJob >= 0) fused_plan_measure(plan, nd, pq.jobs.f[measureJob], pq.jobs.s[measureJob], valueBytes);
  else fused_plan_const_measure(plan, nd, constBits, constDtype, valueBytes);
  return !journal || (columns_cover(journal->colRows.data(), journal->filters.size(), n0) &&
                      fused_plan_filters(plan, journal->filters.data(), journal->filters.size()));
}
void take_queue(PendingQueue &pq, PendingQueue &q) {
  q = pq;
  pq.jobs.count = 0;
  pq.reads.clear();
  pq.writes.clear();
  pq.keep.clear();
  pq.overWait = false;
  if (q.idx) {
    auto jk = t_state->journals.find(q.idx);
// ... 288 lines not shown
    if (ok) {
      const PendingQueue &pq = it->second;
      uint8_t *measureRows = inValues + static_cast<size_t>(valueBytes) * prev;
      if (measureJob >= 0) {
        ok = measure_job_matches(pq.jobs.s[measureJob], measureRows, valueBytes, aggFunc);
      } else {
        auto f = t_state->fills.find(measureRows);
        ok = f != t_state->fills.end() && !f->second.sortIdx && f->second.unit == valueBytes &&
             f->second.bytes == static_cast<size_t>(valueBytes) * pq.n;
        if (ok) {
          constMeasure = true;
          fill = f->second;
          fillAt = f->first;
          constBits = fill.pattern;
        }
      }
      const int constDtype = a.vtype == V_F64 ? Float64 : a.vtype == V_F32 ? Float32 : valueBytes == 8 ? Int64 : (a.vtype == V_I32 ? Int32 : Uint32);
      ok = ok && plan_from_queue(plan, pq, L, dimJob, measureJob, valueBytes, constBits, constDtype, journal, n0);
    }
    if (!ok) {
      materialize_sort(in.IndexVector);
      return false;
    }
    take_queue(it->second, q);
    if (constMeasure) t_state->fills.erase(fillAt);
    drop_sort(in.IndexVector);
  }
  prepare_sort_reduce(device, in, inValues, out, outValues, valueBytes, length, prev);
  const int result = guarded_attempt("fused_sort_reduce_run", [&] {
    return fused_sort_reduce_run(device, plan, nd, constMeasure, constBits, n0, in, inValues, prev, out, outValues, a, stream);
  });
  if (result < 0) {
    {
      DeferLock lock(device);
      launch_queue(stream, q, true);
      if (constMeasure) launch_fill(fillAt, fill);
    }
    g_releaseHeld(device, hold_tag(stream));
    int wide = kFusedUnavailable;
    if (vector_sort_enabled() && vector_sort_layout(in))
      wide = guarded_attempt("fused_sort_reduce_vectors", [&] { return fused_sort_reduce_vectors(device, length, in, inValues, out, outValues, a, stream); });
    if (wide >= 0) {
      ps.fromVectors = true;
      return reduced_sort_done(device, stream, ps, in, inValues, out, outValues, valueBytes, length, aggFunc, wide, nullptr, groups);
    }
    return sort_for_real(device, stream, in, length);
  }
  q.sortIdx = in.IndexVector;
  ps.constMeasure = constMeasure;
  ps.fill = fill;
  ps.fillAt = fillAt;
  return reduced_sort_done(device, stream, ps, in, inValues, out, outValues, valueBytes, length, aggFunc, result, &q, groups);
}

int compact_by_predicate(const uint8_t *pred, uint32_t *indexVector, RecordID **recordIDVectors, int numForeignTables,
                         int n, hipStream_t stream) {
  if (n <= 0) return 0;
  {
    const int device = current_device();
    mem_note_write(device, indexVector, 4ull * static_cast<size_t>(n));
    for (int t = 0; t < numForeignTables; t++) mem_note_write(device, recordIDVectors[t], 8ull * static_cast<size_t>(n));
  }
  const int pad = static_cast<int>(reinterpret_cast<uintptr_t>(pred) & 3);
  const int tiles = pred_tiles(n, pad);
  const int passes = 1 + numForeignTables;
  StreamBuffer wsBuf(CompactSpace::bytes(tiles, passes, 0), stream);
  const CompactSpace cs = clear_compact_space(wsBuf, tiles, passes, 0, stream);
  ARES_LAUNCH("pred_count_kernel", pred_count_kernel, capped_grid(tiles, 256 * 16), kBlock, stream, pred, cs.tileCounts(), pad, n, tiles);
  launch_compaction(cs, pred, indexVector, false, recordIDVectors, pad, n, stream);
  return read_compaction_total(cs, stream);
}

}

using namespace ares;

extern "C" {

size_t AresStreamEvents(int device, void *stream) {
  size_t n = profiler_stream_events(reinterpret_cast<hipStream_t>(stream));
  if (device < 0 || device >= kMaxDevices) return n;
  DeferLock lock(device);
  for (const ErrorCheck &c : t_state->errorChecks) n += c.stream == reinterpret_cast<hipStream_t>(stream);
  return n;
}

void AresTempStats(size_t *handedOutBytes, size_t *cachedBytes) { temp_stats(handedOutBytes, cachedBytes); }

void AresFlushDeferred(int device) {
  int current = 0;
  if (hipGetDevice(&current) != hipSuccess) {
    (void)hipGetLastError();
    return;
  }
  try {
    if (current != device) hip_check(hipSetDevice(device), "hipSetDevice");
    flush_deferred(device);
    if (current != device) (void)hipSetDevice(current);
  } catch (std::exception &e) {
    fprintf(stderr, "Exception happened when flushing deferred transforms: %s\n", e.what());
  }
}

CGoCallResHandle InitIndexVector(uint32_t *indexVector, uint32_t start, int indexVectorLength, void *cudaStream,
                                 int device) {
  ARES_ABI_BEGIN_NOFLUSH(device)
  hipStream_t stream = reinterpret_cast<hipStream_t>(cudaStream);
  begin_batch(device, stream, indexVector, start, indexVectorLength);
  if (!defer_iota(device, stream, indexVector, start, indexVectorLength)) {
    flush_deferred(device);
    DeferLock lock(device);
    launch_init_index(indexVector, start, indexVectorLength, stream);
  }
  ARES_ABI_END("InitIndexVector")
}

CGoCallResHandle UnaryTransform(InputVector input, OutputVector output, uint32_t *indexVector,
                                int indexVectorLength, uint32_t *baseCounts, uint32_t startCount,
                                enum UnaryFunctorType functorType, void *cudaStream, int device) {
  ARES_ABI_BEGIN_NOFLUSH(device)
  resHandle.res = int_result(run_transform(&input, 1, output, indexVector, indexVectorLength, baseCounts,
                                           startCount, functorType, reinterpret_cast<hipStream_t>(cudaStream), device));
  ARES_ABI_END("UnaryTransform")
}

CGoCallResHandle BinaryTransform(InputVector lhs, InputVector rhs, OutputVector output, uint32_t *indexVector,
                                 int indexVectorLength, uint32_t *baseCounts, uint32_t startCount,
                                 enum BinaryFunctorType functorType, void *cudaStream, int device) {
  ARES_ABI_BEGIN_NOFLUSH(device)
  InputVector ins[2] = {lhs, rhs};
  resHandle.res = int_result(run_transform(ins, 2, output, indexVector, indexVectorLength, baseCounts, startCount,
                                           functorType, reinterpret_cast<hipStream_t>(cudaStream), device));
  ARES_ABI_END("BinaryTransform")
}

CGoCallResHandle UnaryFilter(InputVector input, uint32_t *indexVector, uint8_t *predicateVector,
                             int indexVectorLength, RecordID **recordIDVectors, int numForeignTables,
                             uint32_t *baseCounts, uint32_t startCount, enum UnaryFunctorType functorType,
                             void *cudaStream, int device) {
  ARES_ABI_BEGIN_NOFLUSH(device)
  resHandle.res = int_result(run_filter(&input, 1, indexVector, predicateVector, indexVectorLength, recordIDVectors,
                                        numForeignTables, baseCounts, startCount, functorType,
                                        reinterpret_cast<hipStream_t>(cudaStream), device));
  ARES_ABI_END("UnaryFilter")
}

CGoCallResHandle BinaryFilter(InputVector lhs, InputVector rhs, uint32_t *indexVector, uint8_t *predicateVector,
                              int indexVectorLength, RecordID **recordIDVectors, int numForeignTables,
                              uint32_t *baseCounts, uint32_t startCount, enum BinaryFunctorType functorType,
                              void *cudaStream, int device) {
  ARES_ABI_BEGIN_NOFLUSH(device)
  InputVector ins[2] = {lhs, rhs};
  resHandle.res = int_result(run_filter(ins, 2, indexVector, predicateVector, indexVectorLength, recordIDVectors,
                                        numForeignTables, baseCounts, startCount, functorType,
                                        reinterpret_cast<hipStream_t>(cudaStream), device));
  ARES_ABI_END("BinaryFilter")
}

}
```

aresdb_amd/csrc/algo/transform_kernels.hpp:

```cpp
#pragma once

#include <hip/hip_runtime.h>

#include "binding.hpp"
#include "common.hpp"
#include "device_model.hpp"
#include "fast_eval.hpp"
#include "lookback.hpp"

namespace ares {

constexpr int kBlock = 256;
constexpr int kWaves = kBlock / 64;

__global__ __launch_bounds__(kBlock) void init_index_kernel(uint32_t *idx, uint32_t start, int n) {
  const int64_t quads = (static_cast<int64_t>(n) + 3) >> 2;
  for (int64_t q = static_cast<int64_t>(blockIdx.x) * kBlock + threadIdx.x; q < quads;
       q += static_cast<int64_t>(gridDim.x) * kBlock) {
    const int64_t i = q << 2;
    const uint32_t v = start + static_cast<uint32_t>(i);
    if (i + 3 < n && (reinterpret_cast<uintptr_t>(idx) & 15) == 0) {
      *reinterpret_cast<uint4 *>(idx + i) = make_uint4(v, v + 1, v + 2, v + 3);
    } else {
      for (int k = 0; k < 4 && i + k < n; k++) idx[i + k] = v + k;
// ... 759 lines not shown
        *reinterpret_cast<uint32_t *>(pred + i0) = bytes;
      } else {
#pragma unroll
        for (int j = 0; j < 4; j++)
          if (i0 + j >= 0 && i0 + j < n) pred[i0 + j] = static_cast<uint8_t>((kb >> j) & 1u);
      }
    }
#pragma unroll
    for (int off = 32; off > 0; off >>= 1) count += __shfl_xor(count, off);
    if (lane == 0 && count) atomicAdd(tileCounts + tile, count);
    mine += count;
  }
  if (!blockTotals) return;
  __syncthreads();
  if (lane == 0 && mine) atomicAdd(&sTotal, mine);
  __syncthreads();
  if (threadIdx.x == 0) blockTotals[blockIdx.x] = sTotal;
}

template <bool TWO, bool HAS_IN>
__global__ __launch_bounds__(kBlock) void filter_rows_kernel(FastOperands f, FastOperands g, const uint16_t *bitsIn,
                                                             uint16_t *bitsOut, uint16_t *bitsOut2, int n, int numTiles,
                                                             uint32_t *blockTotals) {
  __shared__ uint32_t sTotal[2];
  if (threadIdx.x < 2) sTotal[threadIdx.x] = 0;
  uint32_t mine = 0, mine2 = 0;
  const int lane = threadIdx.x & 63;
  DVal y, z;
  y.bits = f.bbits;
  y.ok = f.bok;
  y = cvt32(y, f.bkind, f.I);
  z.bits = g.bbits;
  z.ok = g.bok;
  z = cvt32(z, g.bkind, g.I);
  for (int tile = blockIdx.x; tile < numTiles; tile += gridDim.x) {
    const int64_t tq = static_cast<int64_t>(tile) * (kBlock * kPQ);
    const size_t word = static_cast<size_t>(tile) * kBlock + threadIdx.x;
    uint32_t alive = 0xFFFFu;
    if (HAS_IN) alive = bitsIn[word];
    uint32_t rows[kPQ][4], vals[kPQ][4], okb[kPQ];
    load_quads<kPQ>(f, tq + threadIdx.x, n, rows, vals, okb);
    uint32_t in[kPQ], kbs[kPQ], kbs2[kPQ];
#pragma unroll
    for (int q = 0; q < kPQ; q++) {
      const int64_t i0 = (tq + threadIdx.x + static_cast<int64_t>(q) * kBlock) * 4;
      in[q] = 0xFu;
      if (i0 + 3 >= n) {
        in[q] = 0;
#pragma unroll
        for (int j = 0; j < 4; j++) in[q] |= (i0 + j < n ? 1u : 0u) << j;
      }
    }
    compare_tile<kPQ>(f, vals, okb, in, y, kbs);
    uint32_t k1 = 0;
#pragma unroll
    for (int q = 0; q < kPQ; q++) k1 |= kbs[q] << (4 * q);
    k1 &= alive;
    bitsOut[word] = static_cast<uint16_t>(k1);
    mine += __popc(k1);
    if (TWO) {
      compare_tile<kPQ>(g, vals, okb, in, z, kbs2);
      uint32_t k2 = 0;
#pragma unroll
      for (int q = 0; q < kPQ; q++) k2 |= kbs2[q] << (4 * q);
      k2 &= k1;
      bitsOut2[word] = static_cast<uint16_t>(k2);
      mine2 += __popc(k2);
    }
  }
#pragma unroll
  for (int off = 32; off > 0; off >>= 1) {
    mine += __shfl_xor(mine, off);
    if (TWO) mine2 += __shfl_xor(mine2, off);
  }
  __syncthreads();
  if (lane == 0) {
    if (mine) atomicAdd(&sTotal[0], mine);
    if (mine2) atomicAdd(&sTotal[1], mine2);
  }
  __syncthreads();
  if (threadIdx.x < 2) blockTotals[2 * blockIdx.x + threadIdx.x] = sTotal[threadIdx.x];
}

__global__ __launch_bounds__(1024) void filter_scan_kernel(const uint32_t *tileCounts, uint32_t *tileOffsets, int numTiles,
                                                           uint32_t *total) {
  constexpr int kPer = 8;
  __shared__ uint32_t sWave[16];
  __shared__ uint32_t sCarry;
  const int lane = threadIdx.x & 63, wave = threadIdx.x >> 6;
  if (threadIdx.x == 0) sCarry = 0;
  __syncthreads();
  for (int base = 0; base < numTiles; base += 1024 * kPer) {
    const int t0 = base + threadIdx.x * kPer;
    uint32_t c[kPer], mine = 0;
#pragma unroll
    for (int k = 0; k < kPer; k++) {
      c[k] = t0 + k < numTiles ? tileCounts[t0 + k] : 0u;
      mine += c[k];
    }
    uint32_t incl = mine;
#pragma unroll
    for (int off = 1; off < 64; off <<= 1) {
      const uint32_t v = __shfl_up(incl, off);
      if (lane >= off) incl += v;
    }
    if (lane == 63) sWave[wave] = incl;
    __syncthreads();
    uint32_t before = sCarry;
    for (int w = 0; w < wave; w++) before += sWave[w];
    uint32_t run = before + incl - mine;
#pragma unroll
    for (int k = 0; k < kPer; k++) {
      if (t0 + k < numTiles) tileOffsets[t0 + k] = run;
      run += c[k];
    }
    __syncthreads();
    if (threadIdx.x == 1023) sCarry = before + incl;
    __syncthreads();
  }
  if (threadIdx.x == 0) {
    tileOffsets[numTiles] = sCarry;
    *total = sCarry;
  }
}

struct CompactWorkspace {
  unsigned int *ticket;
  uint32_t *error;
  const uint32_t *tileOffsets;
  uint32_t *loaded;
};

template <typename PAYLOAD, bool VIRTUAL>
__global__ __launch_bounds__(kBlock) void filter_compact_kernel(const uint8_t *pred, PAYLOAD *data, uint32_t iotaStart, int pad,
                                                                CompactWorkspace ws, int n, int numTiles) {
  __shared__ PAYLOAD sOut[kPTile];
  __shared__ uint32_t sCounts[kPQ * kWaves];
  __shared__ int sTicket;
  const int lane = threadIdx.x & 63, wave = threadIdx.x >> 6;
  for (;;) {
    __syncthreads();
    if (threadIdx.x == 0) sTicket = static_cast<int>(atomicAdd(ws.ticket, 1u));
    __syncthreads();
    const int firstTile = sTicket * kTilesPerTicket;
    if (firstTile >= numTiles) break;
    PAYLOAD rows[kTilesPerTicket][kPQ][4];
    uint32_t keep[kTilesPerTicket];
#pragma unroll
    for (int tt = 0; tt < kTilesPerTicket; tt++) {
      const int tile = firstTile + tt;
      const int64_t tq = static_cast<int64_t>(tile) * (kBlock * kPQ);
      keep[tt] = 0;
#pragma unroll
      for (int q = 0; q < kPQ; q++) {
        const int64_t i0 = (tq + threadIdx.x + static_cast<int64_t>(q) * kBlock) * 4 - pad;
        uint32_t pb = 0;
        if (tile < numTiles && i0 >= 0 && i0 + 3 < n) {
          pb = *reinterpret_cast<const uint32_t *>(pred + i0);
          if (VIRTUAL) {
#pragma unroll
            for (int j = 0; j < 4; j++) rows[tt][q][j] = static_cast<PAYLOAD>(iotaStart + static_cast<uint32_t>(i0) + j);
          } else if (sizeof(PAYLOAD) == 4) {
            const U32x4 r = *reinterpret_cast<const U32x4 *>(data + i0);
#pragma unroll
            for (int j = 0; j < 4; j++) rows[tt][q][j] = static_cast<PAYLOAD>(r.v[j]);
          } else {
// ... 172 lines not shown
```

aresdb_amd/csrc/host/ares_driver.cpp:

```cpp
#include "ares_driver.h"

#include <dlfcn.h>

#include <algorithm>
#include <atomic>
#include <cstdio>
#include <map>
#include <memory>
#include <condition_variable>
#include <mutex>
#include <thread>
#include <cstdlib>
#include <cstring>
#include <stdexcept>
#include <string>
#include <vector>

#include "ares_extensions.h"
#include "ares_memory.h"

namespace {

struct AbiError : std::runtime_error {
  explicit AbiError(const std::string &m) : std::runtime_error(m) {}
};

intptr_t check(CGoCallResHandle h) {
  if (h.pStrErr) {
    std::string msg(h.pStrErr);
    free(const_cast<char *>(h.pStrErr));
    throw AbiError(msg);
  }
  return reinterpret_cast<intptr_t>(h.res);
}

struct AbiLibrary {
  void *algoHandle = nullptr, *memHandle = nullptr;
  decltype(&::InitIndexVector) InitIndexVector;
  decltype(&::HashLookup) HashLookup;
  decltype(&::UnaryTransform) UnaryTransform;
  decltype(&::UnaryFilter) UnaryFilter;
  decltype(&::BinaryTransform) BinaryTransform;
  decltype(&::BinaryFilter) BinaryFilter;
  decltype(&::Sort) Sort;
  decltype(&::Reduce) Reduce;
  decltype(&::HashReduce) HashReduce;
  decltype(&::AresFusedFilterHashReduce) FusedFilterHashReduce = nullptr;
  decltype(&::AresFusedFilterSelect) FusedFilterSelect = nullptr;
  decltype(&::AresFusedFilterJoinSelect) FusedFilterJoinSelect = nullptr;
  decltype(&::AresJoinColumnsRun) JoinColumnsRun = nullptr;
  decltype(&::AresJoinColumnBytes) JoinColumnBytes = nullptr;
  decltype(&::Expand) Expand;
  decltype(&::DeviceAllocate) DeviceAllocate;
  decltype(&::DeviceFree) DeviceFree;
  decltype(&::WaitForCudaStream) WaitForCudaStream;
  decltype(&::HyperLogLog) HyperLogLog;
  decltype(&::GeoBatchIntersects) GeoBatchIntersects;
  decltype(&::WriteGeoShapeDim) WriteGeoShapeDim;
  decltype(&::AsyncCopyDeviceToDevice) AsyncCopyDeviceToDevice;
  decltype(&::AsyncCopyDeviceToHost) AsyncCopyDeviceToHost;
  decltype(&::AsyncCopyHostToDevice) AsyncCopyHostToDevice;
  decltype(&::HostAlloc) HostAlloc;
  decltype(&::HostFree) HostFree;
  void (*NoteWrite)(int, const void *, size_t) = nullptr;
  void (*NoteActivity)() = nullptr;
  void noteWrite(int device, const void *p, size_t bytes) const {
    if (NoteWrite) NoteWrite(device, p, bytes);
    if (NoteActivity) NoteActivity();
  }

  template <typename F>
  void bind(void *handle, const char *name, F &fn) {
    fn = reinterpret_cast<F>(dlsym(handle, name));
    if (!fn) throw AbiError(std::string("missing symbol ") + name);
  }

  AbiLibrary(const char *algoPath, const char *memPath) {
    memHandle = dlopen(memPath, RTLD_NOW | RTLD_LOCAL);
    if (!memHandle) throw AbiError(std::string("dlopen ") + memPath + ": " + dlerror());
    algoHandle = dlopen(algoPath, RTLD_NOW | RTLD_LOCAL);
    if (!algoHandle) throw AbiError(std::string("dlopen ") + algoPath + ": " + dlerror());
    bind(algoHandle, "InitIndexVector", InitIndexVector);
    bind(algoHandle, "HashLookup", HashLookup);
    bind(algoHandle, "UnaryTransform", UnaryTransform);
    bind(algoHandle, "UnaryFilter", UnaryFilter);
    bind(algoHandle, "BinaryTransform", BinaryTransform);
    bind(algoHandle, "BinaryFilter", BinaryFilter);
    bind(algoHandle, "Sort", Sort);
    bind(algoHandle, "Reduce", Reduce);
    bind(algoHandle, "HashReduce", HashReduce);
    bind(algoHandle, "HyperLogLog", HyperLogLog);
    bind(algoHandle, "GeoBatchIntersects", GeoBatchIntersects);
    bind(algoHandle, "WriteGeoShapeDim", WriteGeoShapeDim);
    bind(algoHandle, "Expand", Expand);
    FusedFilterHashReduce = reinterpret_cast<decltype(FusedFilterHashReduce)>(dlsym(algoHandle, "AresFusedFilterHashReduce"));
    FusedFilterSelect = reinterpret_cast<decltype(FusedFilterSelect)>(dlsym(algoHandle, "AresFusedFilterSelect"));
    FusedFilterJoinSelect = reinterpret_cast<decltype(FusedFilterJoinSelect)>(dlsym(algoHandle, "AresFusedFilterJoinSelect"));
    JoinColumnsRun = reinterpret_cast<decltype(JoinColumnsRun)>(dlsym(algoHandle, "AresJoinColumnsRun"));
    JoinColumnBytes = reinterpret_cast<decltype(JoinColumnBytes)>(dlsym(algoHandle, "AresJoinColumnBytes"));
    bind(memHandle, "DeviceAllocate", DeviceAllocate);
    bind(memHandle, "DeviceFree", DeviceFree);
    bind(memHandle, "WaitForCudaStream", WaitForCudaStream);
    bind(memHandle, "AsyncCopyDeviceToDevice", AsyncCopyDeviceToDevice);
    bind(memHandle, "AsyncCopyDeviceToHost", AsyncCopyDeviceToHost);
    bind(memHandle, "AsyncCopyHostToDevice", AsyncCopyHostToDevice);
    bind(memHandle, "HostAlloc", HostAlloc);
    bind(memHandle, "HostFree", HostFree);
    NoteWrite = reinterpret_cast<decltype(NoteWrite)>(dlsym(memHandle, "AresMemNoteWrite"));
    NoteActivity = reinterpret_cast<decltype(NoteActivity)>(dlsym(memHandle, "AresMemNoteActivity"));
  }
  ~AbiLibrary() {
    if (algoHandle) dlclose(algoHandle);
    if (memHandle) dlclose(memHandle);
  }
};

template <typename T>
struct Pod {
  alignas(T) unsigned char bytes[sizeof(T)];
  Pod() { memset(bytes, 0, sizeof(bytes)); }
  T &operator*() { return *reinterpret_cast<T *>(bytes); }
  T *operator->() { return reinterpret_cast<T *>(bytes); }
  const T &get() const { return *reinterpret_cast<const T *>(bytes); }
};
using IV = Pod<InputVector>;
using OV = Pod<OutputVector>;

constexpr int kDimWidths[NUM_DIM_WIDTH] = {16, 8, 4, 2, 1};

int data_type_bytes(int t) {
  switch (t) {
    case Bool: case Int8: case Uint8: return 1;
    case Int16: case Uint16: return 2;
    case Int32: case Uint32: case Float32: return 4;
    case Int64: case Uint64: case Float64: case GeoPoint: return 8;
    case UUID: return 16;
    default: throw AbiError("unknown data type");
  }
}

void dimension_start_offsets(const uint8_t ndw[NUM_DIM_WIDTH], int dimIndex, int64_t capacity, int64_t *valueOff,
                             int64_t *nullOff) {
  int64_t before = 0, all = 0;
  int d = 0, total = 0;
  for (int w = 0; w < NUM_DIM_WIDTH; w++) total += ndw[w];
  for (int w = 0; w < NUM_DIM_WIDTH; w++)
    for (int j = 0; j < ndw[w]; j++, d++) {
      if (d < dimIndex) before += kDimWidths[w];
      all += kDimWidths[w];
    }
  *valueOff = before * capacity;
  *nullOff = all * capacity + static_cast<int64_t>(dimIndex) * capacity;
  (void)total;
}

struct Plan {
  std::vector<AresPlanNode> nodes;
  std::vector<int> filters, foreignFilters, dimNodes, dimTypes;
  int measureNode, aggFunc, measureType;
  bool useHashReduction;
  bool useFusedExtension;
  bool isNonAggregation;
  int limit;
  struct Foreign {
    AresForeignTable t;
    std::vector<VectorPartySlice> slices;
    std::vector<int> dataTypes;
  };
  std::vector<Foreign> foreign;
  bool hasGeo = false;
  AresGeoIntersection geo;

  explicit Plan(const AresQueryPlan &p)
      : nodes(p.nodes, p.nodes + p.numNodes), filters(p.filters, p.filters + p.numFilters),
        foreignFilters(p.foreignFilters, p.foreignFilters + p.numForeignFilters),
        dimNodes(p.dimNodes, p.dimNodes + p.numDims), dimTypes(p.dimTypes, p.dimTypes + p.numDims),
        measureNode(p.measureNode), aggFunc(p.aggFunc), measureType(p.measureType),
        useHashReduction(p.useHashReduction != 0), useFusedExtension(p.useFusedExtension != 0),
        isNonAggregation(p.isNonAggregation != 0), limit(p.limit) {
    for (int i = 0; i < p.numForeignTables; i++) {
      Foreign f;
      f.t = p.foreignTables[i];
      f.slices.assign(f.t.slices, f.t.slices + static_cast<size_t>(f.t.numColumns) * f.t.numBatches);
      f.dataTypes.assign(f.t.dataTypes, f.t.dataTypes + f.t.numColumns);
      foreign.push_back(std::move(f));
    }
    memset(&geo, 0, sizeof(geo));
    if (p.geo) {
      hasGeo = true;
      geo = *p.geo;
    }
  }
  int measureBytes() const { return data_type_bytes(measureType); }
  bool isHLL() const { return aggFunc == AGGR_HLL; }
  int dimRowBytes() const {
    int b = 0;
    for (int t : dimTypes) b += data_type_bytes(t) + 1;
    return b;
  }
};

}

struct AresQuery {
  AbiLibrary *lib;
  Plan plan;
  int device;
  void *stream;
  void *otherStream = nullptr;
  uint8_t ndw[NUM_DIM_WIDTH] = {0, 0, 0, 0, 0};
  std::vector<int> dimVectorIndex;
  int resultSize = 0, resultCapacity = 0;
  uint8_t *dimVec[2] = {nullptr, nullptr};
  uint8_t *measureVec[2] = {nullptr, nullptr};
  uint8_t *hllVector = nullptr;
  uint16_t *hllDimRegIDCount = nullptr;
  size_t hllVectorSize = 0;
  bool isLastBatch = false;
  uint32_t *geoPredicateVec = nullptr;
  int sizeBeforeGeoFilter = 0;
  std::vector<void *> ownedColumns;
  uint64_t *hashVec[2] = {nullptr, nullptr};
  uint32_t *dimIndexVec[2] = {nullptr, nullptr};
  int size = 0;
  uint32_t *indexVec = nullptr;
  uint8_t *predVec = nullptr;
  uint32_t *baseCounts = nullptr;
  uint32_t startRow = 0;
  const VectorPartySlice *columns = nullptr;
  int numColumns = 0;
  std::vector<uint8_t *> stack;
  std::vector<RecordID *> foreignRids;
  long calls = 0, fusedBatches = 0;
  bool fusedDeclined = false;
  struct JoinedTable {
    std::vector<int> columns;
    int first = 0;
  };
  std::vector<JoinedTable> joinedTables;
  std::vector<std::pair<int, int>> joinedLeaves;
  std::unique_ptr<Plan> joinedPlan;
  bool joinColumnsDeclined = false;
  std::vector<VectorPartySlice> extendedColumns;
  std::vector<void *> joinedOutputs;
  int maxBatchSize = 0;
  int batchRows = 0;
  int rowsWritten = 0;
  bool done = false;
  std::vector<std::vector<uint8_t>> hostValues, hostNulls;

  AresQuery(AbiLibrary *l, const AresQueryPlan &p, int dev, void *s) : lib(l), plan(p), device(dev), stream(s) {
    const int n = static_cast<int>(plan.dimTypes.size());
    std::vector<int> order(n);
    for (int i = 0; i < n; i++) order[i] = i;
    std::stable_sort(order.begin(), order.end(), [&](int a, int b) {
      return data_type_bytes(plan.dimTypes[a]) > data_type_bytes(plan.dimTypes[b]);
    });
    dimVectorIndex.assign(n, 0);
    for (int p2 = 0; p2 < n; p2++) dimVectorIndex[order[p2]] = p2;
    for (int t : plan.dimTypes) {
      const int w = data_type_bytes(t);
      for (int k = 0; k < NUM_DIM_WIDTH; k++)
        if (kDimWidths[k] == w) ndw[k]++;
    }
  }

  template <typename T = uint8_t>
  T *alloc(size_t bytes) {
    return reinterpret_cast<T *>(check(lib->DeviceAllocate(bytes ? bytes : 1, device)));
  }
  void release(void *p) {
    if (p) check(lib->DeviceFree(p, device));
  }
  void wait() { check(lib->WaitForCudaStream(stream, device)); }
  void d2d(void *dst, void *src, size_t bytes) {
    if (bytes) check(lib->AsyncCopyDeviceToDevice(dst, src, bytes, stream, device));
  }

  void prepareForFiltering(const VectorPartySlice *cols, int ncols, int n, uint32_t *bc, uint32_t start) {
    columns = cols;
    numColumns = ncols;
    size = n;
    batchRows = n;
    baseCounts = bc;
    startRow = start;
    indexVec = alloc<uint32_t>(static_cast<size_t>(n) * 4);
    predVec = alloc<uint8_t>(static_cast<size_t>(n));
  }

  void prepareForDimAndMeasureEval() {
    if (resultSize + size <= resultCapacity) return;
    const int oldCapacity = resultCapacity;
    resultCapacity = resultSize + size;
    resultCapacity += resultCapacity / 8;
    const int64_t cap = resultCapacity;
    std::vector<int> widths;
    for (int k = 0; k < NUM_DIM_WIDTH; k++)
      for (int j = 0; j < ndw[k]; j++) widths.push_back(kDimWidths[k]);
    {
      uint8_t *old0 = dimVec[0], *old1 = dimVec[1];
      const size_t unit = std::max(plan.dimRowBytes(), 1);
      dimVec[0] = alloc(cap * unit);
      dimVec[1] = alloc(cap * unit);
      if (old0 && resultSize) {
        for (size_t d = 0; d < widths.size(); d++) {
          int64_t nv, nn, ov, on;
          dimension_start_offsets(ndw, static_cast<int>(d), cap, &nv, &nn);
          dimension_start_offsets(ndw, static_cast<int>(d), oldCapacity, &ov, &on);
          d2d(dimVec[0] + nv, old0 + ov, static_cast<size_t>(resultSize) * widths[d]);
          d2d(dimVec[0] + nn, old0 + on, static_cast<size_t>(resultSize));
        }
      }
      if (old0 || old1) wait();
      release(old0);
      release(old1);
    }
    if (plan.isHLL() || !plan.useHashReduction) {
// ... 375 lines not shown
    const int wanted = recordsNeeded();
    if (size != 0 && baseCounts) {
      calls++;
      resultSize = static_cast<int>(check(lib->Expand(dimensionVector(0), dimensionVector(1), baseCounts, indexVec, size, 0, stream, device)));
      std::swap(dimVec[0], dimVec[1]);
    } else {
      resultSize = size;
    }
    if (wanted >= 0 && resultSize > wanted) resultSize = wanted;
  }
  void projectNonAggr() {
    prepareForDimEval();
    evalDimensions();
    expandDimensions();
    wait();
    cleanupBeforeAggregation();
  }
  void postExecNonAggr() {
    const std::vector<int> widths = vectorWidths();
    if (hostValues.empty()) {
      hostValues.resize(widths.size());
      hostNulls.resize(widths.size());
    }
    const size_t n = static_cast<size_t>(resultSize);
    if (n) {
      uint8_t *host = reinterpret_cast<uint8_t *>(check(lib->HostAlloc(n * static_cast<size_t>(plan.dimRowBytes()))));
      uint8_t *to = host;
      for (size_t d = 0; d < widths.size(); d++) {
        int64_t vo, no;
        dimension_start_offsets(ndw, static_cast<int>(d), resultCapacity, &vo, &no);
        check(lib->AsyncCopyDeviceToHost(to, dimVec[0] + vo, n * widths[d], stream, device));
        to += n * widths[d];
      }
      for (size_t d = 0; d < widths.size(); d++) {
        int64_t vo, no;
        dimension_start_offsets(ndw, static_cast<int>(d), resultCapacity, &vo, &no);
        check(lib->AsyncCopyDeviceToHost(to, dimVec[0] + no, n, stream, device));
        to += n;
      }
      wait();
      const uint8_t *from = host;
      for (size_t d = 0; d < widths.size(); d++) {
        hostValues[d].insert(hostValues[d].end(), from, from + n * widths[d]);
        from += n * widths[d];
      }
      for (size_t d = 0; d < widths.size(); d++) {
        hostNulls[d].insert(hostNulls[d].end(), from, from + n);
        from += n;
      }
      check(lib->HostFree(host));
    }
    rowsWritten += resultSize;
    if (recordsNeeded() == 0) done = true;
    size = 0;
  }
  void swapStreams() {
    if (otherStream) std::swap(stream, otherStream);
  }

  bool fusedExpr(int nodeIdx, int outType, AresFusedExpr *e, int *join = nullptr) {
    const AresPlanNode &n = plan.nodes.at(nodeIdx);
    memset(e, 0, sizeof(*e));
    e->outType = static_cast<DataType>(outType);
    auto leafColumn = [&](const AresPlanNode &c, InputVector *iv) {
      if (c.kind != ARES_NODE_COLUMN || c.table < 0 || c.table > static_cast<int>(plan.foreign.size())) return false;
      if (c.table != 0 && !join) return false;
      if (join) *join = c.table - 1;
      memcpy(iv, &columnInput(c, false).get(), sizeof(InputVector));
      return true;
    };
    if (n.kind == ARES_NODE_COLUMN) {
      e->arity = 1;
      e->functor = Noop;
      return leafColumn(n, &e->lhs);
    }
    if (n.kind != ARES_NODE_BINARY) return false;
    const AresPlanNode &l = plan.nodes.at(n.lhs), &r = plan.nodes.at(n.rhs);
    if (r.kind != ARES_NODE_CONST_INT && r.kind != ARES_NODE_CONST_FLOAT) return false;
    if (!leafColumn(l, &e->lhs)) return false;
    memcpy(&e->rhs, &constantInput(r).get(), sizeof(InputVector));
    e->arity = 2;
    e->functor = n.op;
    return true;
  }

  bool runBatchFused(const VectorPartySlice *cols, int ncols, int n) {
    if (!plan.useFusedExtension || !plan.useHashReduction || fusedDeclined || !lib->FusedFilterHashReduce) return false;
    if (plan.hasGeo || plan.isHLL()) return false;
    if (!plan.foreign.empty() || !plan.foreignFilters.empty() || baseCounts) return false;
    if (plan.dimNodes.empty() || plan.dimNodes.size() > 4 || plan.filters.size() > 4) return false;
    columns = cols;
    numColumns = ncols;
    Pod<AresFusedQuery> q;
    q->numFilters = static_cast<int>(plan.filters.size());
    for (size_t i = 0; i < plan.filters.size(); i++)
      if (!fusedExpr(plan.filters[i], Bool, &q->filters[i])) return false;
    q->numDims = static_cast<int>(plan.dimNodes.size());
    for (size_t i = 0; i < plan.dimNodes.size(); i++) {
      if (data_type_bytes(plan.dimTypes[i]) != 4) return false;
      if (!fusedExpr(plan.dimNodes[i], plan.dimTypes[i], &q->dims[dimVectorIndex[i]])) return false;
    }
    if (!fusedExpr(plan.measureNode, plan.measureType, &q->measure)) return false;
    q->aggFunc = static_cast<AggregateFunction>(plan.aggFunc);
    size = n;
    prepareForDimAndMeasureEval();
    calls++;
    CGoCallResHandle h = lib->FusedFilterHashReduce(&q.get(), n, dimensionVector(0), measureVec[0], resultSize,
                                                    dimensionVector(1), measureVec[1], stream, device);
    if (h.pStrErr && strncmp(h.pStrErr, "not fusable", 11) == 0) {
      free(const_cast<char *>(h.pStrErr));
      fusedDeclined = true;
      size = 0;
      return false;
    }
    resultSize = static_cast<int>(check(h));
    wait();
    releaseInputColumns();
    swapResultBuffers();
    fusedBatches++;
    return true;
  }

  bool runBatchFusedSelect(const VectorPartySlice *cols, int ncols, int n) {
    const bool joins = !plan.foreign.empty() || !plan.foreignFilters.empty();
    if (!plan.useFusedExtension || fusedDeclined || !(joins ? lib->FusedFilterJoinSelect != nullptr : lib->FusedFilterSelect != nullptr)) return false;
    if (baseCounts || plan.hasGeo) return false;
    if (plan.foreign.size() > 2 || plan.foreignFilters.size() > 4) return false;
    if (plan.dimNodes.empty() || plan.dimNodes.size() > 8 || plan.filters.size() > 4) return false;
    columns = cols;
    numColumns = ncols;
    CGoCallResHandle h;
    if (joins) {
      Pod<AresFusedJoinSelect> q;
      q->numFilters = static_cast<int>(plan.filters.size());
      for (size_t i = 0; i < plan.filters.size(); i++)
        if (!fusedExpr(plan.filters[i], Bool, &q->filters[i])) return false;
      q->numJoins = static_cast<int>(plan.foreign.size());
      for (size_t k = 0; k < plan.foreign.size(); k++) {
        AresPlanNode key;
        memset(&key, 0, sizeof(key));
        key.kind = ARES_NODE_COLUMN;
        key.column = plan.foreign[k].t.joinColumn;
        memcpy(&q->joins[k].key, &columnInput(key).get(), sizeof(InputVector));
        memcpy(&q->joins[k].index, &plan.foreign[k].t.index, sizeof(CuckooHashIndex));
      }
      q->numForeignFilters = static_cast<int>(plan.foreignFilters.size());
      for (size_t i = 0; i < plan.foreignFilters.size(); i++)
        if (!fusedExpr(plan.foreignFilters[i], Bool, &q->foreignFilters[i], &q->foreignFilterJoin[i]) || q->foreignFilterJoin[i] < 0) return false;
      q->numDims = static_cast<int>(plan.dimNodes.size());
      for (size_t i = 0; i < plan.dimNodes.size(); i++)
        if (!fusedExpr(plan.dimNodes[i], plan.dimTypes[i], &q->dims[dimVectorIndex[i]], &q->dimJoin[dimVectorIndex[i]])) return false;
      size = n;
      batchRows = n;
      prepareForDimEval();
      calls++;
      h = lib->FusedFilterJoinSelect(&q.get(), n, recordsNeeded(), dimensionVector(0), stream, device);
    } else {
      Pod<AresFusedSelect> q;
      q->numFilters = static_cast<int>(plan.filters.size());
      for (size_t i = 0; i < plan.filters.size(); i++)
        if (!fusedExpr(plan.filters[i], Bool, &q->filters[i])) return false;
      q->numDims = static_cast<int>(plan.dimNodes.size());
      for (size_t i = 0; i < plan.dimNodes.size(); i++)
        if (!fusedExpr(plan.dimNodes[i], plan.dimTypes[i], &q->dims[dimVectorIndex[i]])) return false;
      size = n;
      batchRows = n;
      prepareForDimEval();
      calls++;
      h = lib->FusedFilterSelect(&q.get(), n, recordsNeeded(), dimensionVector(0), stream, device);
    }
    if (h.pStrErr && strncmp(h.pStrErr, "not fusable", 11) == 0) {
      free(const_cast<char *>(h.pStrErr));
      fusedDeclined = true;
      size = 0;
      return false;
    }
    resultSize = static_cast<int>(check(h));
    wait();
    releaseInputColumns();
    postExecNonAggr();
    fusedBatches++;
    return true;
  }

  void runBatchNonAggr(const VectorPartySlice *cols, int ncols, int n, uint32_t *bc, uint32_t start) {
    if (done) {
      ownedColumns.clear();
      return;
    }
    baseCounts = bc;
    if (!runBatchFusedSelect(cols, ncols, n)) {
      prepareForFiltering(cols, ncols, n, bc, start);
      preExec();
      filter();
      join();
      projectNonAggr();
      postExecNonAggr();
    }
    swapStreams();
  }

  void runBatch(const VectorPartySlice *cols, int ncols, int n, uint32_t *bc, uint32_t start) {
    if (plan.isNonAggregation) {
      runBatchNonAggr(cols, ncols, n, bc, start);
      return;
    }
    baseCounts = bc;
    struct PlanSwap {
      Plan &a, *b;
      PlanSwap(Plan &a_, Plan *b_) : a(a_), b(b_) {
        if (b) std::swap(a, *b);
      }
      ~PlanSwap() {
        if (b) std::swap(a, *b);
      }
    } joined(plan, resolveJoinedColumns(cols, ncols, n) ? joinedPlan.get() : nullptr);
    if (joined.b) {
      cols = extendedColumns.data();
      ncols = static_cast<int>(extendedColumns.size());
    }
    if (runBatchFused(cols, ncols, n)) {
      swapStreams();
      return;
    }
    prepareForFiltering(cols, ncols, n, bc, start);
    preExec();
    filter();
    join();
    project();
    reduce();
    postExec();
    swapStreams();
  }

  void planJoinedColumns() {
    joinedPlan.reset();
    joinedTables.clear();
    joinedLeaves.clear();
    if (plan.isNonAggregation || plan.foreign.empty() || !lib->JoinColumnsRun || !lib->JoinColumnBytes) return;
    if (plan.hasGeo && plan.geo.pointTable != 0) return;
    const int numNodes = static_cast<int>(plan.nodes.size());
    std::vector<char> reached(plan.nodes.size(), 0);
    bool ok = true;
    auto walk = [&](int root, bool foreignAllowed, auto &&self) -> void {
      if (root < 0 || root >= numNodes) {
        ok = false;
        return;
      }
      const AresPlanNode &n = plan.nodes[root];
      reached[root] = 1;
      if (n.kind == ARES_NODE_COLUMN && n.table != 0 && !foreignAllowed) ok = false;
      if (n.kind == ARES_NODE_UNARY || n.kind == ARES_NODE_BINARY) self(n.lhs, foreignAllowed, self);
      if (n.kind == ARES_NODE_BINARY) self(n.rhs, foreignAllowed, self);
    };
    for (int f : plan.filters) walk(f, false, walk);
    for (int f : plan.foreignFilters) walk(f, true, walk);
    for (size_t i = 0; i < plan.dimNodes.size(); i++)
      if (!(plan.hasGeo && plan.geo.dimIndex == static_cast<int>(i))) walk(plan.dimNodes[i], true, walk);
    walk(plan.measureNode, true, walk);
    if (!ok) return;
    joinedTables.assign(plan.foreign.size(), JoinedTable());
    std::vector<std::pair<int, size_t>> leaves;
    for (int i = 0; i < numNodes; i++) {
      const AresPlanNode &n = plan.nodes[i];
      if (!reached[i] || n.kind != ARES_NODE_COLUMN || n.table == 0) continue;
      if (n.table < 0 || n.table > static_cast<int>(plan.foreign.size())) return;
      const Plan::Foreign &ft = plan.foreign[n.table - 1];
      if (n.column < 0 || n.column >= ft.t.numColumns) return;
      const int t = ft.dataTypes[n.column];
      if (!(t == Int8 || t == Uint8 || t == Int16 || t == Uint16 || t == Int32 || t == Uint32 || t == Float32)) return;
      std::vector<int> &list = joinedTables[n.table - 1].columns;
      size_t at = std::find(list.begin(), list.end(), n.column) - list.begin();
      if (at == list.size()) list.push_back(n.column);
      if (list.size() > 4) return;
      leaves.emplace_back(i, at);
    }
    int total = 0;
    for (JoinedTable &jt : joinedTables) {
      jt.first = total;
      total += static_cast<int>(jt.columns.size());
    }
    joinedPlan.reset(new Plan(plan));
    for (const auto &leaf : leaves) {
      AresPlanNode &n = joinedPlan->nodes[leaf.first];
      joinedLeaves.emplace_back(leaf.first, joinedTables[n.table - 1].first + static_cast<int>(leaf.second));
      n.table = 0;
    }
    joinedPlan->filters.insert(joinedPlan->filters.end(), plan.foreignFilters.begin(), plan.foreignFilters.end());
    joinedPlan->foreignFilters.clear();
    joinedPlan->foreign.clear();
  }

  bool resolveJoinedColumns(const VectorPartySlice *cols, int ncols, int n) {
    if (!joinedPlan || joinColumnsDeclined || baseCounts || n <= 0) return false;
    columns = cols;
    numColumns = ncols;
    int total = 0;
    for (const JoinedTable &jt : joinedTables) total += static_cast<int>(jt.columns.size());
    extendedColumns.assign(cols, cols + ncols);
    extendedColumns.resize(static_cast<size_t>(ncols + total));
    for (size_t k = 0; k < joinedTables.size(); k++) {
      const JoinedTable &jt = joinedTables[k];
      if (jt.columns.empty()) continue;
      Pod<AresJoinColumns> q;
      for (int f : plan.filters)
        if (q->numFilters < 4 && fusedExpr(f, Bool, &q->filters[q->numFilters]) && q->filters[q->numFilters].arity == 2) q->numFilters++;
      AresPlanNode leaf;
      memset(&leaf, 0, sizeof(leaf));
      leaf.kind = ARES_NODE_COLUMN;
      leaf.column = plan.foreign[k].t.joinColumn;
      memcpy(&q->join.key, &columnInput(leaf).get(), sizeof(InputVector));
      memcpy(&q->join.index, &plan.foreign[k].t.index, sizeof(CuckooHashIndex));
      q->numColumns = static_cast<int>(jt.columns.size());
      leaf.table = static_cast<int>(k) + 1;
      for (size_t c = 0; c < jt.columns.size(); c++) {
        leaf.column = jt.columns[c];
        memcpy(&q->columns[c].column, &columnInput(leaf, false).get(), sizeof(InputVector));
        const size_t bytes = lib->JoinColumnBytes(n, static_cast<DataType>(plan.foreign[k].dataTypes[leaf.column]));
        joinedOutputs.push_back(alloc(bytes));
        q->columns[c].out = static_cast<uint8_t *>(joinedOutputs.back());
      }
      calls++;
      CGoCallResHandle h = lib->JoinColumnsRun(&q.get(), n, &extendedColumns[static_cast<size_t>(ncols + jt.first)], stream, device);
      if (h.pStrErr && strncmp(h.pStrErr, "not fusable", 11) == 0) {
        free(const_cast<char *>(h.pStrErr));
        joinColumnsDeclined = true;
        for (void *p : joinedOutputs) release(p);
        joinedOutputs.clear();
        foreignSliceArrays.clear();
        return false;
      }
      check(h);
    }
    foreignSliceArrays.clear();
    for (const auto &leafAt : joinedLeaves) joinedPlan->nodes[leafAt.first].column = ncols + leafAt.second;
    return true;
  }
};

namespace {
void set_err(char *err, int errLen, const char *msg) {
  if (err && errLen > 0) {
    strncpy(err, msg, static_cast<size_t>(errLen) - 1);
    err[errLen - 1] = 0;
  }
}
}

extern "C" {

void *AresDriverOpen(const char *libalgorithmPath, const char *libmemPath, char *err, int errLen) {
  try {
    return new AbiLibrary(libalgorithmPath, libmemPath);
  } catch (std::exception &e) {
    set_err(err, errLen, e.what());
    return nullptr;
  }
}

void AresDriverClose(void *driver) { delete static_cast<AbiLibrary *>(driver); }

AresQuery *AresQueryCreate(void *driver, const AresQueryPlan *plan, int device, void *stream, char *err, int errLen) {
  try {
    return new AresQuery(static_cast<AbiLibrary *>(driver), *plan, device, stream);
  } catch (std::exception &e) {
    set_err(err, errLen, e.what());
    return nullptr;
  }
}

int AresQueryRunBatch(AresQuery *q, const VectorPartySlice *columns, int numColumns, int size, uint32_t *baseCounts,
                      uint32_t startRow, char *err, int errLen) {
  try {
    q->runBatch(columns, numColumns, size, baseCounts, startRow);
    return 0;
  } catch (std::exception &e) {
    set_err(err, errLen, e.what());
    try {
      q->cleanupBeforeAggregation();
    } catch (...) {
    }
    return -1;
  }
}

int AresQueryRunResidentBatches(AresQuery *q, const VectorPartySlice *columns, int numColumns, const int *sizes, int numBatches,
                                char *err, int errLen) {
  for (int b = 0; b < numBatches; b++) {
    q->ownedColumns.clear();
    q->isLastBatch = false;
    const int rc = AresQueryRunBatch(q, columns + static_cast<size_t>(b) * numColumns, numColumns, sizes[b], nullptr, 0, err, errLen);
    if (rc != 0) return rc;
  }
  return 0;
}

int AresQueryResultSize(const AresQuery *q) { return q->plan.isNonAggregation ? q->rowsWritten : q->resultSize; }
int AresQueryDone(const AresQuery *q) { return q->done ? 1 : 0; }
void AresQuerySetMaxBatchSize(AresQuery *q, int rows) { q->maxBatchSize = rows > 0 ? rows : 0; }
int AresQueryResultCapacity(const AresQuery *q) { return q->resultCapacity; }
uint8_t *AresQueryDimensionVector(const AresQuery *q) { return q->dimVec[0]; }
uint8_t *AresQueryMeasureVector(const AresQuery *q) { return q->measureVec[0]; }
long AresQueryNumCalls(const AresQuery *q) { return q->calls; }
long AresQueryNumFusedBatches(const AresQuery *q) { return q->fusedBatches; }
void AresQuerySetLastBatch(AresQuery *q, int isLast) { q->isLastBatch = isLast != 0; }
void AresQuerySetJoinColumns(AresQuery *q, int on) {
  if (on) q->planJoinedColumns();
  else q->joinedPlan.reset();
}
void AresQuerySetSecondStream(AresQuery *q, void *stream) { q->otherStream = stream; }
void AresQueryAdoptColumns(AresQuery *q, void *const *allocations, int count) {
  q->ownedColumns.assign(allocations, allocations + count);
}
int64_t AresQueryHLLVectorSize(const AresQuery *q) { return static_cast<int64_t>(q->hllVectorSize); }

int AresQueryFetchHLL(AresQuery *q, uint16_t *regCounts, uint8_t *hllVector, char *err, int errLen) {
  try {
    const int n = q->resultSize;
    if (n && q->hllDimRegIDCount)
      check(q->lib->AsyncCopyDeviceToHost(regCounts, q->hllDimRegIDCount, static_cast<size_t>(n) * 2, q->stream, q->device));
    if (n && q->hllVector)
      check(q->lib->AsyncCopyDeviceToHost(hllVector, q->hllVector, q->hllVectorSize, q->stream, q->device));
    q->wait();
    return 0;
  } catch (std::exception &e) {
    set_err(err, errLen, e.what());
    return -1;
  }
}

int AresQueryFetch(AresQuery *q, uint8_t *dims, uint8_t *measures, char *err, int errLen) {
  try {
    if (q->plan.isNonAggregation) {
      uint8_t *out = dims;
      for (const std::vector<uint8_t> &v : q->hostValues) out = std::copy(v.begin(), v.end(), out);
      for (const std::vector<uint8_t> &v : q->hostNulls) out = std::copy(v.begin(), v.end(), out);
      return 0;
    }
    const int n = q->resultSize;
    std::vector<int> widths;
    for (int k = 0; k < NUM_DIM_WIDTH; k++)
      for (int j = 0; j < q->ndw[k]; j++) widths.push_back(kDimWidths[k]);
    uint8_t *out = dims;
    for (size_t d = 0; d < widths.size() && n; d++) {
      int64_t vo, no;
      dimension_start_offsets(q->ndw, static_cast<int>(d), q->resultCapacity, &vo, &no);
      check(q->lib->AsyncCopyDeviceToHost(out, q->dimVec[0] + vo, static_cast<size_t>(n) * widths[d], q->stream, q->device));
      out += static_cast<size_t>(n) * widths[d];
    }
    for (size_t d = 0; d < widths.size() && n; d++) {
      int64_t vo, no;
      dimension_start_offsets(q->ndw, static_cast<int>(d), q->resultCapacity, &vo, &no);
      check(q->lib->AsyncCopyDeviceToHost(out, q->dimVec[0] + no, static_cast<size_t>(n), q->stream, q->device));
      out += n;
    }
    if (n && measures) check(q->lib->AsyncCopyDeviceToHost(measures, q->measureVec[0], static_cast<size_t>(n) * q->plan.measureBytes(),
                                               q->stream, q->device));
    q->wait();
    return 0;
  } catch (std::exception &e) {
    set_err(err, errLen, e.what());
    return -1;
  }
}

void AresQueryDestroy(AresQuery *q) {
  if (!q) return;
  try {
    q->cleanupBeforeAggregation();
    q->releaseAll();
  } catch (...) {
  }
  delete q;
}
// ... 738 lines not shown
```

include/ares_extensions.h:

```cpp
#ifndef ARES_EXTENSIONS_H_
#define ARES_EXTENSIONS_H_

#include <stddef.h>
#include <stdint.h>

#include "ares_algorithm.h"

#ifdef __cplusplus
extern "C" {
#endif

void AresProfilerEnable(int on);
size_t AresProfilerReport(char *buf, size_t len);

void AresReloadEnv(void);

size_t AresRtcWait(long *counters);

void AresFlushDeferred(int device);
void AresMemSetFlushHook(void (*hook)(int device));

typedef struct {
  void (*flush)(int device);
  void (*on_wait)(int device, void *stream);
  uintptr_t (*on_free)(int device, void *ptr, size_t bytes);
  void (*on_access)(int device, const void *ptr, size_t bytes);
} AresDeferralHooks;
void AresMemSetDeferralHooks(const AresDeferralHooks *hooks);
void AresMemReleaseHeld(int device, uintptr_t tag);

typedef struct {
  size_t size;
  void (*on_write)(int device, const void *ptr, size_t bytes);
  void (*on_stream_destroy)(int device, void *stream);
  void (*trim)(int device);
} AresMemAuxHooks;
void AresMemSetAuxHooks(const AresMemAuxHooks *hooks);
void AresMemTrimCache(int device);
void AresMemNoteWrite(int device, const void *ptr, size_t bytes);
void AresMemEnableWriteTracking(void);

void AresMemNoteActivity(void);
void AresMemEnableActivityTracking(void);

void AresMemStats(int device, size_t *liveBytes, size_t *liveBlocks, size_t *heldBlocks, size_t *parkedBytes);
void AresMemDriverCalls(int device, size_t *mallocs, size_t *frees, size_t *trims);
size_t AresMemStreamEvents(int device, void *stream);
size_t AresStreamEvents(int device, void *stream);
void AresTempStats(size_t *handedOutBytes, size_t *cachedBytes);

void AresHllPreaggStats(unsigned long long *counters);

typedef struct {
  InputVector lhs, rhs;
  int arity;
  int functor;
  enum DataType outType;
} AresFusedExpr;

typedef struct {
  int numFilters;
  AresFusedExpr filters[4];
  int numDims;
  AresFusedExpr dims[4];
  AresFusedExpr measure;
  enum AggregateFunction aggFunc;
} AresFusedQuery;

CGoCallResHandle AresFusedFilterHashReduce(const AresFusedQuery *query, int batchRows, DimensionVector prevKeys,
                                           uint8_t *prevValues, int prevSize, DimensionVector outKeys,
                                           uint8_t *outValues, void *cudaStream, int device);

typedef struct {
  int numFilters;
  AresFusedExpr filters[4];
  int numDims;
  AresFusedExpr dims[8];
} AresFusedSelect;

CGoCallResHandle AresFusedFilterSelect(const AresFusedSelect *query, int batchRows, int limit ,
                                       DimensionVector outKeys, void *cudaStream, int device);
void AresSelectStats(unsigned long long *counters);
void AresSelectRunStats(unsigned long long *counters);

typedef struct {
  InputVector key;
  CuckooHashIndex index;
} AresFusedJoin;

typedef struct {
  int numFilters;
  AresFusedExpr filters[4];
  int numJoins;
  AresFusedJoin joins[2];
  int numForeignFilters;
  AresFusedExpr foreignFilters[4];
  int foreignFilterJoin[4];
  int numDims;
  AresFusedExpr dims[8];
  int dimJoin[8];
} AresFusedJoinSelect;

CGoCallResHandle AresFusedFilterJoinSelect(const AresFusedJoinSelect *query, int batchRows, int limit ,
                                           DimensionVector outKeys, void *cudaStream, int device);
void AresSelectJoinStats(unsigned long long *counters);

typedef struct {
  InputVector column;
  uint8_t *out;
} AresJoinedColumn;

typedef struct {
  int numFilters;
  AresFusedExpr filters[4];
  AresFusedJoin join;
  int numColumns;
  AresJoinedColumn columns[4];
} AresJoinColumns;

size_t AresJoinColumnBytes(int rows, enum DataType type);
CGoCallResHandle AresJoinColumnsRun(const AresJoinColumns *q, int batchRows, VectorPartySlice *outSlices, void *cudaStream,
                                    int device);
void AresJoinColumnStats(unsigned long long *counters);

#ifdef __cplusplus
}
#endif
#endif
```

Before: 89.64 billion rows/s.

## Precompute next batch's filter bitmaps on the other stream behind the current scan

After: 91.35 billion rows/s (median of 6 runs). 1.02x the previous value.

```diff
diff --git a/aresdb_amd/abi.py b/aresdb_amd/abi.py
--- a/aresdb_amd/abi.py
+++ b/aresdb_amd/abi.py
@@ -337,6 +337,24 @@
         self._algo.AresJoinColumnStats(c)
         return {"batches": int(c[0]), "declined": int(c[1]), "rows": int(c[2]), "probed": int(c[3])}
 
+    @property
+    def has_filter_ahead(self):
+        return hasattr(self._algo, "AresFilterAhead")
+
+    def filter_ahead(self, exprs, batch_rows, stream=None, behind=None, device=0):
+        fn = self._algo.AresFilterAhead
+        fn.argtypes = [C.POINTER(FusedExpr), C.c_int, C.c_int, _S, _S, _I]
+        fn.restype = CGoCallResHandle
+        arr = (FusedExpr * max(len(exprs), 1))(*exprs)
+        return _check(fn(arr, len(exprs), int(batch_rows), stream, behind, device))
+
+    def filter_ahead_stats(self):
+        c = (C.c_ulonglong * 5)()
+        self._algo.AresFilterAheadStats.argtypes, self._algo.AresFilterAheadStats.restype = [C.POINTER(C.c_ulonglong)], None
+        self._algo.AresFilterAheadStats(c)
+        return {"requests": int(c[0]), "behind_scan": int(c[1]), "handed_out": int(c[2]), "mismatched": int(c[3]),
+                "invalidated": int(c[4])}
+
     def select_run_stats(self):
         c = (C.c_ulonglong * 2)()
         self._algo.AresSelectRunStats.argtypes, self._algo.AresSelectRunStats.restype = [C.POINTER(C.c_ulonglong)], None
diff --git a/aresdb_amd/csrc/algo/common.hpp b/aresdb_amd/csrc/algo/common.hpp
--- a/aresdb_amd/csrc/algo/common.hpp
+++ b/aresdb_amd/csrc/algo/common.hpp
@@ -64,6 +64,13 @@
                                    const DimensionVector &out, uint8_t *outValues, int valueBytes, int length, int aggFunc,
                                    int *groups);
 void invalidate_filter_journal(int device, const uint32_t *indexVector);
+void filter_ahead_behind_scan(int device, hipStream_t stream);
+void filter_ahead_after_aggregation(int device, hipStream_t stream) noexcept;
+struct FilterAheadAtReturn {
+  int device;
+  hipStream_t stream;
+  ~FilterAheadAtReturn() { filter_ahead_after_aggregation(device, stream); }
+};
 bool global_table_forced();
 bool deferral_hooks_active();
 void grouped_note_write(int device, const void *ptr, size_t bytes);
diff --git a/aresdb_amd/csrc/algo/hash_reduce.hip b/aresdb_amd/csrc/algo/hash_reduce.hip
--- a/aresdb_amd/csrc/algo/hash_reduce.hip
+++ b/aresdb_amd/csrc/algo/hash_reduce.hip
@@ -119,6 +119,7 @@
                                        enum AggregateFunction aggFunc, void *cudaStream, int device) {
   ARES_ABI_BEGIN_NOFLUSH(device)
   hipStream_t stream = reinterpret_cast<hipStream_t>(cudaStream);
+  const FilterAheadAtReturn aheadAtReturn{device, stream};
   if (length > 0) {
     settle_dimension_vector(device, inputKeys);
     const DimLayoutD inLayout = make_dim_layout(inputKeys.NumDimsPerDimWidth);
diff --git a/aresdb_amd/csrc/algo/hash_reduce_lds.hip b/aresdb_amd/csrc/algo/hash_reduce_lds.hip
--- a/aresdb_amd/csrc/algo/hash_reduce_lds.hip
+++ b/aresdb_amd/csrc/algo/hash_reduce_lds.hip
@@ -705,6 +705,7 @@
     else if (batchRows > 0)                                                                                            \
       ARES_LAUNCH("hr_fused_scan_kernel", hr_fused_scan_kernel<ND>, streams, kThreads, stream, plan,                   \
                   static_cast<uint32_t>(prevSize), a, batchRows, ws);                                                  \
+    filter_ahead_behind_scan(device, stream);      \
     if (leanMerge || tableMerge)                                                                                       \
       rtc_merge_launch(leanMerge ? leanMerge : tableMerge, plan, prevKeys.DimValues, prevCapacity, prevValues,         \
                        static_cast<uint32_t>(prevSize), outKeys.DimValues, outCapacity, outValues, ws, stream, imagePtr, \
@@ -723,6 +724,7 @@
       default:
         if (batchRows > 0 && lean) rtc_scan_launch(lean, leanKind, plan, static_cast<uint32_t>(prevSize), batchRows, ws, stream);
         else if (batchRows > 0 && table) rtc_scan_launch(table, RTC_SCAN_TABLE, plan, static_cast<uint32_t>(prevSize), batchRows, ws, stream);
+        filter_ahead_behind_scan(device, stream);
         rtc_merge_launch(leanMerge ? leanMerge : tableMerge, plan, prevKeys.DimValues, prevCapacity, prevValues, static_cast<uint32_t>(prevSize),
                          outKeys.DimValues, outCapacity, outValues, ws, stream, imagePtr, result_slot());
         break;
diff --git a/aresdb_amd/csrc/algo/hll.hip b/aresdb_amd/csrc/algo/hll.hip
--- a/aresdb_amd/csrc/algo/hll.hip
+++ b/aresdb_amd/csrc/algo/hll.hip
@@ -647,6 +647,7 @@
                                         uint8_t **hllVectorPtr, size_t *hllVectorSizePtr,
                                         uint16_t **hllDimRegIDCountPtr, void *cudaStream, int device) {
   ARES_ABI_BEGIN(device)
+  const FilterAheadAtReturn aheadAtReturn{device, reinterpret_cast<hipStream_t>(cudaStream)};
   settle_dimension_vector(device, prevDimOut);
   settle_dimension_vector(device, curDimOut);
   {
diff --git a/aresdb_amd/csrc/algo/sort_reduce.hip b/aresdb_amd/csrc/algo/sort_reduce.hip
--- a/aresdb_amd/csrc/algo/sort_reduce.hip
+++ b/aresdb_amd/csrc/algo/sort_reduce.hip
@@ -932,6 +932,7 @@
                         uint8_t *outputValues, int valueBytes, int length, enum AggregateFunction aggFunc,
                         void *cudaStream, int device) {
   ARES_ABI_BEGIN_NOFLUSH(device)
+  const FilterAheadAtReturn aheadAtReturn{device, reinterpret_cast<hipStream_t>(cudaStream)};
   {
     int groups = 0;
     if (reduce_without_dimensions(device, inputKeys, inputValues, outputKeys, outputValues, valueBytes, length, aggFunc,
diff --git a/aresdb_amd/csrc/algo/transform.hip b/aresdb_amd/csrc/algo/transform.hip
--- a/aresdb_amd/csrc/algo/transform.hip
+++ b/aresdb_amd/csrc/algo/transform.hip
@@ -3,6 +3,7 @@
 #include <dlfcn.h>
 
 #include <algorithm>
+#include <atomic>
 #include <map>
 #include <memory>
 #include <mutex>
@@ -269,6 +270,22 @@
   std::shared_ptr<StreamBuffer> ws;
 };
 
+struct AheadSlot {
+  uint32_t *words = nullptr;
+  hipEvent_t done = nullptr;
+};
+constexpr int kAheadGridCap = 512;
+struct AheadRequest {
+  hipStream_t stream, behind;
+  int n0 = 0, count = 0, grid = 0;
+  FastOperands f[kFusedFilters];
+  uint32_t colRows[kFusedFilters];
+  std::shared_ptr<StreamBuffer> bits[kFusedFilters];
+  std::shared_ptr<AheadSlot> slot;
+  bool launched = false;
+  int handed = 0;
+};
+
 struct DeferState {
   std::mutex mutex;
   int device = -1;
@@ -282,6 +299,7 @@
   std::map<uint8_t *, PendingFill> fills;
   std::map<const uint32_t *, PendingSort> sorts;
   std::map<hipStream_t, std::vector<RunExpansion>> expansions;
+  std::map<hipStream_t, std::shared_ptr<AheadRequest>> ahead;
   std::vector<ErrorCheck> errorChecks;
   std::vector<uint32_t *> errorSlots;
   bool errorSeen = false;
@@ -1197,6 +1215,169 @@
          a.bbits == b.bbits && a.bok == b.bok;
 }
 
+bool filter_ahead_enabled() {
+  static EnvSwitch<bool> on("ARES_FILTER_AHEAD", [](const char *e) { return !(e && e[0] == '0'); });
+  return on.get();
+}
+enum { AHEAD_REQUESTS, AHEAD_BEHIND_SCAN, AHEAD_HANDED, AHEAD_MISMATCH, AHEAD_INVALIDATED, AHEAD_COUNTERS };
+std::atomic<unsigned long long> g_aheadStats[AHEAD_COUNTERS];
+
+std::mutex g_aheadSlotMutex;
+std::map<std::pair<int, hipStream_t>, std::vector<AheadSlot>> g_aheadSlots;
+void destroy_ahead_slot(AheadSlot &s) {
+  if (s.done) (void)hipEventDestroy(s.done);
+  if (s.words) (void)hipHostFree(s.words);
+  s = AheadSlot{};
+}
+std::shared_ptr<AheadSlot> take_ahead_slot(int device, hipStream_t stream) {
+  AheadSlot s;
+  {
+    std::lock_guard<std::mutex> lock(g_aheadSlotMutex);
+    std::vector<AheadSlot> &idle = g_aheadSlots[{device, stream}];
+    if (!idle.empty()) {
+      s = idle.back();
+      idle.pop_back();
+    }
+  }
+  if (!s.words) {
+    try {
+      hip_check(hipHostMalloc(reinterpret_cast<void **>(&s.words), sizeof(uint32_t) * 2 * kAheadGridCap * kFusedFilters,
+                              hipHostMallocPortable | hipHostMallocMapped),
+                "hipHostMalloc");
+      hip_check(hipEventCreateWithFlags(&s.done, hipEventDisableTiming), "hipEventCreate");
+    } catch (...) {
+      destroy_ahead_slot(s);
+      throw;
+    }
+  }
+  return std::shared_ptr<AheadSlot>(new AheadSlot(s), [device, stream](AheadSlot *p) {
+    {
+      std::lock_guard<std::mutex> lock(g_aheadSlotMutex);
+      auto it = g_aheadSlots.find({device, stream});
+      if (it != g_aheadSlots.end()) {
+        it->second.push_back(*p);
+        *p = AheadSlot{};
+      }
+    }
+    destroy_ahead_slot(*p);
+    delete p;
+  });
+}
+void ahead_slots_stream_gone(int device, hipStream_t stream) {
+  std::vector<AheadSlot> idle;
+  {
+    std::lock_guard<std::mutex> lock(g_aheadSlotMutex);
+    auto it = g_aheadSlots.find({device, stream});
+    if (it == g_aheadSlots.end()) return;
+    idle.swap(it->second);
+    g_aheadSlots.erase(it);
+  }
+  for (AheadSlot &s : idle) destroy_ahead_slot(s);
+}
+
+int ahead_gate_mode() {
+  static EnvSwitch<int> mode("ARES_FILTER_AHEAD_GATE", [](const char *e) { return e && e[0] >= '0' && e[0] <= '3' ? e[0] - '0' : 0; });
+  return mode.get();
+}
+void launch_ahead(AheadRequest &r, bool gate) {
+  if (r.launched) return;
+  if (gate && r.behind && r.behind != r.stream && ahead_gate_mode() != 0) {
+    hipEvent_t reached;
+    hip_check(hipEventCreateWithFlags(&reached, hipEventDisableTiming | (ahead_gate_mode() == 2 ? hipEventReleaseToDevice : 0u)), "hipEventCreate");
+    hipError_t e = hipEventRecord(reached, r.behind);
+    if (e == hipSuccess) e = hipStreamWaitEvent(r.stream, reached, 0);
+    (void)hipEventDestroy(reached);
+    hip_check(e, "hipStreamWaitEvent");
+  }
+  const int tiles = pred_tiles(r.n0, 0);
+  for (int j = 0; j < r.count; j++) {
+    auto kernel = j ? &filter_rows_ahead_kernel<true> : &filter_rows_ahead_kernel<false>;
+    ARES_LAUNCH("filter_rows_ahead_kernel", kernel, r.grid, kBlock, r.stream, r.f[j],
+                j ? r.bits[j - 1]->as<uint16_t>() : static_cast<const uint16_t *>(nullptr), r.bits[j]->as<uint16_t>(), r.n0, tiles,
+                r.slot->words + static_cast<size_t>(2 * kAheadGridCap) * j);
+  }
+  hip_check(hipEventRecord(r.slot->done, r.stream), "hipEventRecord");
+  mem_note_activity();
+  r.launched = true;
+}
+void drop_ahead(std::map<hipStream_t, std::shared_ptr<AheadRequest>>::iterator it, int why) {
+  g_aheadStats[why]++;
+  t_state->ahead.erase(it);
+}
+void drop_ahead_of_stream(int device, hipStream_t stream, int why) {
+  DeferLock lock(device);
+  auto it = t_state->ahead.find(stream);
+  if (it != t_state->ahead.end()) drop_ahead(it, why);
+}
+void drop_ahead_touching(const ByteRange &r) {
+  for (auto it = t_state->ahead.begin(); it != t_state->ahead.end();) {
+    const AheadRequest &q = *it->second;
+    bool hit = false;
+    for (int j = q.handed; j < q.count; j++) hit = hit || column_overlaps(q.f[j], q.colRows[j], r);
+    if (!hit) {
+      ++it;
+      continue;
+    }
+    if (q.launched) t_syncAfterUnlock.push_back(q.stream);
+    drop_ahead(it++, AHEAD_INVALIDATED);
+  }
+}
+void launch_ahead_behind(int device, hipStream_t stream, bool behindScan) {
+  if (!defer_available() || (behindScan && ahead_gate_mode() == 3)) return;
+  DeferLock lock(device);
+  for (auto it = t_state->ahead.begin(); it != t_state->ahead.end();) {
+    AheadRequest &r = *it->second;
+    if (r.launched || r.behind != stream) {
+      ++it;
+      continue;
+    }
+    try {
+      launch_ahead(r, behindScan);
+      if (behindScan) g_aheadStats[AHEAD_BEHIND_SCAN]++;
+      ++it;
+    } catch (std::exception &) {
+      drop_ahead(it++, AHEAD_INVALIDATED);
+    }
+  }
+}
+
+int filter_ahead_request(int device, const AresFusedExpr *filters, int numFilters, int n0, hipStream_t stream, hipStream_t behind) {
+  if (!fuse_available() || !row_space_enabled() || !filter_ahead_enabled() || !filters || n0 <= 0) return 0;
+  auto r = std::make_shared<AheadRequest>();
+  r->stream = stream;
+  r->behind = behind;
+  r->n0 = n0;
+  for (int k = 0; k < numFilters && k < kFusedFilters; k++) {
+    const AresFusedExpr &e = filters[k];
+    if (e.arity != 2 || e.lhs.Type != VectorPartyInput || e.rhs.Type != ConstantInput) break;
+    InputVector ins[2] = {e.lhs, e.rhs};
+    EvalParams p;
+    CallTemps temps;
+    build_params(ins, 2, stream, nullptr, nullptr, 0, e.functor, p, temps);
+    FastOperands f;
+    if (is_wide(p.a.kind) || !fast_operands(p, f, true) || p.a.length < static_cast<uint32_t>(n0)) break;
+    f.idx = nullptr;
+    f.pad = 0;
+    f.streaming = 1;
+    r->f[k] = f;
+    r->colRows[k] = p.a.length;
+    r->count++;
+  }
+  if (r->count == 0) return 0;
+  const int tiles = pred_tiles(n0, 0);
+  r->grid = capped_grid(tiles, std::min(kAheadGridCap, compute_units(device)));
+  const size_t bitBytes = static_cast<size_t>(tiles) * kBlock * sizeof(uint16_t);
+  DeferLock lock(device);
+  auto old = t_state->ahead.find(stream);
+  if (old != t_state->ahead.end()) drop_ahead(old, AHEAD_MISMATCH);
+  r->slot = take_ahead_slot(device, stream);
+  for (int j = 0; j < r->count; j++) r->bits[j] = std::make_shared<StreamBuffer>(bitBytes, stream);
+  if (!behind) launch_ahead(*r, false);
+  t_state->ahead[stream] = r;
+  g_aheadStats[AHEAD_REQUESTS]++;
+  return r->count;
+}
+
 bool row_space_eligible(int device, hipStream_t stream, const uint32_t *indexVector, int n, uint32_t colRows) {
   if (!fuse_available() || !row_space_enabled()) return false;
   DeferLock lock(device);
@@ -1222,9 +1403,12 @@
   bool two = false;
   FastOperands g = f;
   uint64_t generation = 0;
+  std::shared_ptr<AheadSlot> aheadSlot;
+  size_t aheadWords = 0;
   {
     DeferLock lock(device);
     auto ins = t_state->compactions.find(indexVector);
+    auto ahead = t_state->ahead.find(stream);
     {
       auto jr = t_state->journals.find(indexVector);
       const size_t journalled = (jr != t_state->journals.end() && jr->second.valid) ? jr->second.filters.size() : 0;
@@ -1232,6 +1416,17 @@
       const bool next = ins != t_state->compactions.end() && !ins->second.todo.empty() && ins->second.stream == stream &&
                         ins->second.applied + ins->second.todo.size() + 1 == journalled && ins->second.lastCount == n;
       if (!first && !next) return -1;
+      if (ahead != t_state->ahead.end()) {
+        const AheadRequest &r = *ahead->second;
+        const int j = r.handed;
+        const bool fits = r.launched && j < r.count && !keep && same_filter(r.f[j], f) && r.colRows[j] == colRows &&
+                          (first ? (j == 0 && r.n0 == n)
+                                 : (j > 0 && r.n0 == ins->second.n0 && ins->second.bits == r.bits[j - 1] && !ins->second.predicted.valid));
+        if (!fits) {
+          drop_ahead(ahead, AHEAD_MISMATCH);
+          ahead = t_state->ahead.end();
+        }
+      }
     }
     if (ins == t_state->compactions.end()) {
       PendingCompact fresh{};
@@ -1248,7 +1443,16 @@
     FilterShape shape{f.akind, f.functor, f.I, f.bkind, f.bbits, f.bok, !c.todo.empty() && same_column(c.todo.back().f, f)};
     const size_t k = h.current.size();
     h.current.push_back(shape);
-    if (c.predicted.valid && same_filter(c.predicted.g, f)) {
+    if (ahead != t_state->ahead.end()) {
+      AheadRequest &r = *ahead->second;
+      const int j = r.handed++;
+      aheadSlot = r.slot;
+      aheadWords = static_cast<size_t>(2 * kAheadGridCap) * j;
+      grid = r.grid;
+      bits1 = r.bits[j];
+      if (r.handed == r.count) t_state->ahead.erase(ahead);
+      g_aheadStats[AHEAD_HANDED]++;
+    } else if (c.predicted.valid && same_filter(c.predicted.g, f)) {
       const int count = c.predicted.count;
       c.todo.push_back(LazyFilter{f, colRows, pred, n, keep});
       c.bits = c.predicted.bits;
@@ -1259,40 +1463,43 @@
       return count;
     }
     c.predicted = PredictedFilter{};
-    if (k + 1 < h.previous.size() && h.previous[k].same_as(shape) && h.previous[k + 1].sameColumnAsPrevious &&
-        h.previous[k + 1].akind == f.akind && c.applied + c.todo.size() + 2 <= static_cast<size_t>(kFusedFilters)) {
-      const FilterShape &nx = h.previous[k + 1];
-      g.functor = nx.functor;
-      g.I = nx.I;
-      g.bkind = nx.bkind;
-      g.bbits = nx.bbits;
-      g.bok = nx.bok;
-      two = true;
-    }
-    const int tiles = pred_tiles(c.n0, 0);
-    const bool hasIn = static_cast<bool>(c.bits);
-    auto kernel = two ? (hasIn ? &filter_rows_kernel<true, true> : &filter_rows_kernel<true, false>)
-                      : (hasIn ? &filter_rows_kernel<false, true> : &filter_rows_kernel<false, false>);
-    {
-      const int resident = resident_blocks(device, reinterpret_cast<const void *>(kernel), kBlock), cus = compute_units(device);
-      const int perUnit = std::max(1, std::min(resident / cus - 1, 6));
-      grid = capped_grid(tiles, std::min(kGridCap, cus * perUnit));
-    }
-    const size_t bitBytes = static_cast<size_t>(tiles) * kBlock * sizeof(uint16_t);
-    bits1 = std::make_shared<StreamBuffer>(bitBytes, stream);
-    if (two) bits2 = std::make_shared<StreamBuffer>(bitBytes, stream);
-    uint32_t *hostPartials = reinterpret_cast<uint32_t *>(pinned_words());
-    ARES_LAUNCH("filter_rows_kernel", kernel, grid, kBlock, stream, f, g,
-                hasIn ? c.bits->as<uint16_t>() : static_cast<const uint16_t *>(nullptr), bits1->as<uint16_t>(),
-                two ? bits2->as<uint16_t>() : static_cast<uint16_t *>(nullptr), c.n0, tiles, hostPartials);
+    if (!aheadSlot) {
+      if (k + 1 < h.previous.size() && h.previous[k].same_as(shape) && h.previous[k + 1].sameColumnAsPrevious &&
+          h.previous[k + 1].akind == f.akind && c.applied + c.todo.size() + 2 <= static_cast<size_t>(kFusedFilters)) {
+        const FilterShape &nx = h.previous[k + 1];
+        g.functor = nx.functor;
+        g.I = nx.I;
+        g.bkind = nx.bkind;
+        g.bbits = nx.bbits;
+        g.bok = nx.bok;
+        two = true;
+      }
+      const int tiles = pred_tiles(c.n0, 0);
+      const bool hasIn = static_cast<bool>(c.bits);
+      auto kernel = two ? (hasIn ? &filter_rows_kernel<true, true> : &filter_rows_kernel<true, false>)
+                        : (hasIn ? &filter_rows_kernel<false, true> : &filter_rows_kernel<false, false>);
+      {
+        const int resident = resident_blocks(device, reinterpret_cast<const void *>(kernel), kBlock), cus = compute_units(device);
+        const int perUnit = std::max(1, std::min(resident / cus - 1, 6));
+        grid = capped_grid(tiles, std::min(kGridCap, cus * perUnit));
+      }
+      const size_t bitBytes = static_cast<size_t>(tiles) * kBlock * sizeof(uint16_t);
+      bits1 = std::make_shared<StreamBuffer>(bitBytes, stream);
+      if (two) bits2 = std::make_shared<StreamBuffer>(bitBytes, stream);
+      uint32_t *hostPartials = reinterpret_cast<uint32_t *>(pinned_words());
+      ARES_LAUNCH("filter_rows_kernel", kernel, grid, kBlock, stream, f, g,
+                  hasIn ? c.bits->as<uint16_t>() : static_cast<const uint16_t *>(nullptr), bits1->as<uint16_t>(),
+                  two ? bits2->as<uint16_t>() : static_cast<uint16_t *>(nullptr), c.n0, tiles, hostPartials);
+    }
     c.todo.push_back(LazyFilter{f, colRows, pred, n, keep});
     c.bits = bits1;
     c.lastCount = -1;
     generation = ++t_state->filterGeneration;
     c.generation = generation;
   }
-  hip_check(hipStreamSynchronize(stream), "hipStreamSynchronize");
-  const volatile uint32_t *parts = reinterpret_cast<const volatile uint32_t *>(pinned_words());
+  if (aheadSlot) hip_check(hipEventSynchronize(aheadSlot->done), "hipEventSynchronize");
+  else hip_check(hipStreamSynchronize(stream), "hipStreamSynchronize");
+  const volatile uint32_t *parts = aheadSlot ? aheadSlot->words + aheadWords : reinterpret_cast<const volatile uint32_t *>(pinned_words());
   uint32_t count = 0, count2 = 0;
   for (int b = 0; b < grid; b++) {
     count += parts[2 * b];
@@ -1455,6 +1662,7 @@
     const int counted = run_filter_rows(device, stream, f, indexVector, pred, n, p.a.length, virtualIdx, decoded);
     if (counted >= 0) return counted;
   }
+  if (defer_available()) drop_ahead_of_stream(device, stream, AHEAD_MISMATCH);
   if (rowSpace) {
     mem_note_write(device, pred, static_cast<size_t>(n));
     DeferLock lock(device);
@@ -1540,6 +1748,7 @@
     }
     retire_fills(r, true);
     forget_run_expansions(r);
+    drop_ahead_touching(r);
     for (auto it = t_state->journals.begin(); it != t_state->journals.end();) {
       const bool dead = journal_touched(it->first, it->second, r, nullptr);
       bool kept = false;
@@ -1628,6 +1837,7 @@
       }
     }
     forget_run_expansions(r);
+    drop_ahead_touching(r);
     materialize_fills(&r, &t_syncAfterUnlock);
     materialize_limbo(&r, &released);
     for (auto it = t_state->compactions.begin(); it != t_state->compactions.end();) {
@@ -1686,6 +1896,14 @@
       for (auto it = t_state->iotas.begin(); it != t_state->iotas.end();)
         it = it->second.stream == stream ? t_state->iotas.erase(it) : std::next(it);
       t_state->filterHistory.erase(stream);
+      for (auto it = t_state->ahead.begin(); it != t_state->ahead.end();) {
+        if (it->second->stream != stream && it->second->behind != stream) {
+          ++it;
+          continue;
+        }
+        if (it->second->stream == stream && it->second->launched) t_syncAfterUnlock.push_back(stream);
+        drop_ahead(it++, AHEAD_INVALIDATED);
+      }
       for (auto &kv : t_state->fills)
         if (kv.second.stream == stream) kv.second.streamGone = true;
       for (size_t i = 0; i < t_state->errorChecks.size();) {
@@ -1694,12 +1912,21 @@
       }
     }
     profiler_stream_gone(stream);
+    ahead_slots_stream_gone(device, stream);
     if (g_releaseHeld) g_releaseHeld(device, hold_tag(stream));
     stream_cache_purge(device, stream);
   } catch (std::exception &e) {
     fprintf(stderr, "Exception happened when handling a stream destruction: %s\n", e.what());
   }
 }
+}
+
+void filter_ahead_behind_scan(int device, hipStream_t stream) { launch_ahead_behind(device, stream, true); }
+void filter_ahead_after_aggregation(int device, hipStream_t stream) noexcept {
+  try {
+    launch_ahead_behind(device, stream, false);
+  } catch (std::exception &) {
+  }
 }
 
 void launch_pending_writers(int device, const void *ptr, size_t bytes) {
@@ -2154,7 +2381,21 @@
   if (device < 0 || device >= kMaxDevices) return n;
   DeferLock lock(device);
   for (const ErrorCheck &c : t_state->errorChecks) n += c.stream == reinterpret_cast<hipStream_t>(stream);
+  for (const auto &kv : t_state->ahead) n += kv.first == reinterpret_cast<hipStream_t>(stream) && kv.second->launched;
   return n;
+}
+
+CGoCallResHandle AresFilterAhead(const AresFusedExpr *filters, int numFilters, int batchRows, void *cudaStream, void *behindStream,
+                                 int device) {
+  ARES_ABI_BEGIN_NOFLUSH(device)
+  resHandle.res = int_result(filter_ahead_request(device, filters, numFilters, batchRows, reinterpret_cast<hipStream_t>(cudaStream),
+                                                  reinterpret_cast<hipStream_t>(behindStream)));
+  ARES_ABI_END("AresFilterAhead")
+}
+
+void AresFilterAheadStats(unsigned long long *counters) {
+  if (!counters) return;
+  for (int i = 0; i < AHEAD_COUNTERS; i++) counters[i] = g_aheadStats[i].load(std::memory_order_relaxed);
 }
 
 void AresTempStats(size_t *handedOutBytes, size_t *cachedBytes) { temp_stats(handedOutBytes, cachedBytes); }
diff --git a/aresdb_amd/csrc/algo/transform_kernels.hpp b/aresdb_amd/csrc/algo/transform_kernels.hpp
--- a/aresdb_amd/csrc/algo/transform_kernels.hpp
+++ b/aresdb_amd/csrc/algo/transform_kernels.hpp
@@ -865,6 +865,89 @@
   if (threadIdx.x < 2) blockTotals[2 * blockIdx.x + threadIdx.x] = sTotal[threadIdx.x];
 }
 
+template <bool HAS_IN>
+__global__ __launch_bounds__(kBlock) void filter_rows_ahead_kernel(FastOperands f, const uint16_t *bitsIn, uint16_t *bitsOut, int n,
+                                                                   int numTiles, uint32_t *blockTotals) {
+  __shared__ uint32_t sTotal;
+  if (threadIdx.x == 0) sTotal = 0;
+  uint32_t mine = 0;
+  const int lane = threadIdx.x & 63;
+  DVal y;
+  y.bits = f.bbits;
+  y.ok = f.bok;
+  y = cvt32(y, f.bkind, f.I);
+  constexpr int kPair = 2;
+  const uint32_t rowsN = static_cast<uint32_t>(n);
+  for (int tile = blockIdx.x; tile < numTiles; tile += gridDim.x) {
+    const size_t word = static_cast<size_t>(tile) * kBlock + threadIdx.x;
+    uint32_t k1 = 0;
+#pragma unroll 1
+    for (int half = 0; half < kPQ / kPair; half++) {
+      uint32_t vals[kPair][4], okb[kPair], in[kPair], kbs[kPair];
+#pragma unroll
+      for (int q = 0; q < kPair; q++) {
+        const uint32_t i0 = ((static_cast<uint32_t>(tile) * kPQ + kPair * half + q) * kBlock + threadIdx.x) * 4u;
+        const bool full = i0 + 3 < rowsN;
+        const uint32_t r0 = i0 < rowsN ? i0 : 0u;
+        in[q] = 0xFu;
+        if (!full) {
+          in[q] = 0;
+#pragma unroll
+          for (int j = 0; j < 4; j++) in[q] |= (i0 + j < rowsN ? 1u : 0u) << j;
+        }
+        if (f.step == 2) {
+          const uint16_t *v16 = reinterpret_cast<const uint16_t *>(f.vals);
+          uint32_t raw[4];
+          if (full) {
+            const PU32x2 v = *reinterpret_cast<const PU32x2 *>(v16 + r0);
+            raw[0] = v.v[0] & 0xFFFFu; raw[1] = v.v[0] >> 16; raw[2] = v.v[1] & 0xFFFFu; raw[3] = v.v[1] >> 16;
+          } else {
+#pragma unroll
+            for (int j = 0; j < 4; j++) raw[j] = v16[i0 + j < rowsN ? i0 + j : 0u];
+          }
+#pragma unroll
+          for (int j = 0; j < 4; j++) vals[q][j] = f.akind == K_I32 ? static_cast<uint32_t>(static_cast<int32_t>(static_cast<int16_t>(raw[j]))) : raw[j];
+        } else if (f.step == 1) {
+          const uint8_t *v8 = reinterpret_cast<const uint8_t *>(f.vals);
+          uint32_t raw[4];
+          if (full) {
+            const uint32_t v = reinterpret_cast<const PU32s1 *>(v8 + r0)->v;
+            raw[0] = v & 0xFFu; raw[1] = (v >> 8) & 0xFFu; raw[2] = (v >> 16) & 0xFFu; raw[3] = v >> 24;
+          } else {
+#pragma unroll
+            for (int j = 0; j < 4; j++) raw[j] = v8[i0 + j < rowsN ? i0 + j : 0u];
+          }
+#pragma unroll
+          for (int j = 0; j < 4; j++) vals[q][j] = f.akind == K_I32 ? static_cast<uint32_t>(static_cast<int32_t>(static_cast<int8_t>(raw[j]))) : raw[j];
+        } else if (full) {
+          typedef uint32_t V4 __attribute__((ext_vector_type(4)));
+          typedef V4 V4a __attribute__((aligned(4)));
+          const V4 v = __builtin_nontemporal_load(reinterpret_cast<const V4a *>(f.vals + r0));
+          vals[q][0] = v.x; vals[q][1] = v.y; vals[q][2] = v.z; vals[q][3] = v.w;
+        } else {
+#pragma unroll
+          for (int j = 0; j < 4; j++) vals[q][j] = f.vals[i0 + j < rowsN ? i0 + j : 0u];
+        }
+        uint32_t window = 0xFFFFu;
+        if (f.nulls) window = reinterpret_cast<const PU16 *>(f.nulls + ((r0 + f.bitOff) >> 3))->v;
+        okb[q] = (window >> ((r0 + f.bitOff) & 7u)) & 0xFu;
+      }
+      compare_tile<kPair>(f, vals, okb, in, y, kbs);
+#pragma unroll
+      for (int q = 0; q < kPair; q++) k1 |= kbs[q] << (4 * (kPair * half + q));
+    }
+    if (HAS_IN) k1 &= bitsIn[word];
+    bitsOut[word] = static_cast<uint16_t>(k1);
+    mine += __popc(k1);
+  }
+#pragma unroll
+  for (int off = 32; off > 0; off >>= 1) mine += __shfl_xor(mine, off);
+  __syncthreads();
+  if (lane == 0 && mine) atomicAdd(&sTotal, mine);
+  __syncthreads();
+  if (threadIdx.x < 2) blockTotals[2 * blockIdx.x + threadIdx.x] = threadIdx.x == 0 ? sTotal : 0u;
+}
+
 __global__ __launch_bounds__(1024) void filter_scan_kernel(const uint32_t *tileCounts, uint32_t *tileOffsets, int numTiles,
                                                            uint32_t *total) {
   constexpr int kPer = 8;
diff --git a/aresdb_amd/csrc/host/ares_driver.cpp b/aresdb_amd/csrc/host/ares_driver.cpp
--- a/aresdb_amd/csrc/host/ares_driver.cpp
+++ b/aresdb_amd/csrc/host/ares_driver.cpp
@@ -50,6 +50,7 @@
   decltype(&::AresFusedFilterJoinSelect) FusedFilterJoinSelect = nullptr;
   decltype(&::AresJoinColumnsRun) JoinColumnsRun = nullptr;
   decltype(&::AresJoinColumnBytes) JoinColumnBytes = nullptr;
+  decltype(&::AresFilterAhead) FilterAhead = nullptr;
   decltype(&::Expand) Expand;
   decltype(&::DeviceAllocate) DeviceAllocate;
   decltype(&::DeviceFree) DeviceFree;
@@ -98,6 +99,7 @@
     FusedFilterJoinSelect = reinterpret_cast<decltype(FusedFilterJoinSelect)>(dlsym(algoHandle, "AresFusedFilterJoinSelect"));
     JoinColumnsRun = reinterpret_cast<decltype(JoinColumnsRun)>(dlsym(algoHandle, "AresJoinColumnsRun"));
     JoinColumnBytes = reinterpret_cast<decltype(JoinColumnBytes)>(dlsym(algoHandle, "AresJoinColumnBytes"));
+    FilterAhead = reinterpret_cast<decltype(FilterAhead)>(dlsym(algoHandle, "AresFilterAhead"));
     bind(memHandle, "DeviceAllocate", DeviceAllocate);
     bind(memHandle, "DeviceFree", DeviceFree);
     bind(memHandle, "WaitForCudaStream", WaitForCudaStream);
@@ -233,6 +235,8 @@
   std::vector<RecordID *> foreignRids;
   long calls = 0, fusedBatches = 0;
   bool fusedDeclined = false;
+  const VectorPartySlice *nextColumns = nullptr;
+  int nextNumColumns = 0, nextSize = 0;
   struct JoinedTable {
     std::vector<int> columns;
     int first = 0;
@@ -774,6 +778,30 @@
     e->arity = 2;
     e->functor = n.op;
     return true;
+  }
+
+  void requestFilterAhead() {
+    if (!lib->FilterAhead || !nextColumns || nextSize <= 0 || plan.filters.empty()) return;
+    if (plan.useFusedExtension && !fusedDeclined) return;
+    if (joinedPlan || !plan.foreign.empty() || !plan.foreignFilters.empty() || plan.hasGeo || baseCounts) return;
+    std::vector<Pod<AresFusedExpr>> exprs(plan.filters.size());
+    for (size_t i = 0; i < plan.filters.size(); i++) {
+      const AresPlanNode &n = plan.nodes.at(plan.filters[i]);
+      if (n.kind != ARES_NODE_BINARY) return;
+      const AresPlanNode &l = plan.nodes.at(n.lhs), &r = plan.nodes.at(n.rhs);
+      if (l.kind != ARES_NODE_COLUMN || l.table != 0 || l.column < 0 || l.column >= nextNumColumns) return;
+      if (r.kind != ARES_NODE_CONST_INT && r.kind != ARES_NODE_CONST_FLOAT) return;
+      IV lhs;
+      lhs->Vector.VP = nextColumns[l.column];
+      lhs->Type = VectorPartyInput;
+      memcpy(&exprs[i]->lhs, &lhs.get(), sizeof(InputVector));
+      memcpy(&exprs[i]->rhs, &constantInput(r).get(), sizeof(InputVector));
+      exprs[i]->arity = 2;
+      exprs[i]->functor = n.op;
+      exprs[i]->outType = Bool;
+    }
+    static_assert(sizeof(Pod<AresFusedExpr>) == sizeof(AresFusedExpr), "an array of boxes is an array of expressions");
+    check(lib->FilterAhead(&exprs[0].get(), static_cast<int>(exprs.size()), nextSize, otherStream ? otherStream : stream, stream, device));
   }
 
   bool runBatchFused(const VectorPartySlice *cols, int ncols, int n) {
@@ -920,6 +948,7 @@
     filter();
     join();
     project();
+    requestFilterAhead();
     reduce();
     postExec();
     swapStreams();
@@ -1081,7 +1110,12 @@
   for (int b = 0; b < numBatches; b++) {
     q->ownedColumns.clear();
     q->isLastBatch = false;
+    q->nextColumns = b + 1 < numBatches ? columns + static_cast<size_t>(b + 1) * numColumns : nullptr;
+    q->nextNumColumns = numColumns;
+    q->nextSize = b + 1 < numBatches ? sizes[b + 1] : 0;
     const int rc = AresQueryRunBatch(q, columns + static_cast<size_t>(b) * numColumns, numColumns, sizes[b], nullptr, 0, err, errLen);
+    q->nextColumns = nullptr;
+    q->nextSize = 0;
     if (rc != 0) return rc;
   }
   return 0;
diff --git a/include/ares_extensions.h b/include/ares_extensions.h
--- a/include/ares_extensions.h
+++ b/include/ares_extensions.h
@@ -71,6 +71,10 @@
                                            uint8_t *prevValues, int prevSize, DimensionVector outKeys,
                                            uint8_t *outValues, void *cudaStream, int device);
 
+CGoCallResHandle AresFilterAhead(const AresFusedExpr *filters, int numFilters, int batchRows, void *cudaStream,
+                                 void *behindStream, int device);
+void AresFilterAheadStats(unsigned long long *counters);
+
 typedef struct {
   int numFilters;
   AresFusedExpr filters[4];
```
